# Saro00/DGN

Hardware: AMD Instinct MI355X
Metric: dgn_layer_fwd_bwd_edges_per_sec (higher is better)
Workload: dtype f32; 1 GPU; c2: ZINC-12k (12000 molecules, one batch), DGN towers: 5 towers, hidden 70, mean max min dir1-av dir1-dx x identity amplification attenuation; edges_per_gpu=586426, nodes_per_gpu=275167, parallelism=single GPU, step=edge weights + layer forward + backward

## Files before the change

dgn_amd/csrc/dgn_abi.hip:

```cpp
#include <hip/hip_runtime.h>

#include <atomic>
#include <cstdarg>
#include <cstdio>
#include <cstdlib>
#include <cstring>
#include <mutex>

#include "dgn_common.hpp"

namespace dgn {
namespace {
thread_local char g_err[512] = "";
}

void set_error(const char* fmt, ...) {
    va_list ap;
    va_start(ap, fmt);
    vsnprintf(g_err, sizeof(g_err), fmt, ap);
    va_end(ap);
}

namespace {
__global__ void zero_rows_kernel(int64_t rows, int64_t width, int64_t ld, float* __restrict__ p) {
// ... 30 lines not shown
hipError_t allow_lds(LdsOptIn& done, int bytes, const void* const* kernels, int n_kernels) {
    int dev = 0;
    hipError_t e = hipGetDevice(&dev);
    if (e != hipSuccess) return e;
    const unsigned long long bit = dev >= 0 && dev < 64 ? 1ull << dev : 0;
    if (done.load(std::memory_order_acquire) & bit) return hipSuccess;
    for (int i = 0; i < n_kernels; ++i) {
        e = hipFuncSetAttribute(kernels[i], hipFuncAttributeMaxDynamicSharedMemorySize, bytes);
        if (e != hipSuccess) return e;
    }
    done.fetch_or(bit, std::memory_order_release);
    return hipSuccess;
}

int n_cus() {
    static int cus = 0;
    if (!cus) {
        int dev = 0;
        hipDeviceProp_t prop;
        if (hipGetDevice(&dev) != hipSuccess || hipGetDeviceProperties(&prop, dev) != hipSuccess) return 256;
        cus = prop.multiProcessorCount > 0 ? prop.multiProcessorCount : 256;
    }
    return cus;
}

int hip_fail(hipError_t e, const char* what) {
    set_error("HIP error %d (%s) in %s", (int)e, hipGetErrorString(e), what);
    return DGN_ERR_HIP;
}
}

namespace dgn {
namespace {
struct OptDef { const char* name; const char* env; int64_t def; bool presence; };
const OptDef kOpts[OPT_COUNT] = {
    {"blk_lds_kb", "DGN_BLK_LDS_KB", 13, false},
    {"blk_min_nodes", "DGN_BLK_MIN_NODES", 131072, false},
    {"bwd_rows_per_wave", "DGN_BWD_ROWS_PER_WAVE", 4, false},
    {"tile_gemm", "DGN_TILE_GEMM", -1, false},
    {"tile_wgrad", "DGN_TILE_WGRAD", -1, false},
    {"no_zmask", "DGN_NO_ZMASK", 0, true},
    {"linear_small_min_waves", "DGN_LINEAR_SMALL_MIN_WAVES", 8, false},
    {"graph_bwd_tiles", "DGN_GRAPH_BWD_TILES", 0, false},
    {"odd_direct", "DGN_ODD_DIRECT", 1, false},
    {"bn_from_wgrad", "DGN_BN_FROM_WGRAD", 1, false},
    {"mix_bwd_fused", "DGN_MIX_BWD_FUSED", 1, false},
    {"blk_lds_pad_kb", "DGN_BLK_LDS_PAD_KB", 0, false},
    {"lin_wreg", "DGN_LIN_WREG", 3, false},
    {"bd_bwd_fused", "DGN_BD_BWD_FUSED", 1, false},
    {"bn_stats_fused", "DGN_BN_STATS_FUSED", 1, false},
    {"ew_big_min", "DGN_EW_BIG_MIN", 1 << 19, false},
    {"ew_separate", "DGN_EW_SEPARATE", 0, true},
    {"ew_no_flat8", "DGN_EW_NO_FLAT8", 0, true},
};
std::atomic<int64_t> g_opt[OPT_COUNT];
std::once_flag g_opt_once;
void init_options() {
    for (int i = 0; i < OPT_COUNT; ++i) {
        const char* e = getenv(kOpts[i].env);
        g_opt[i].store(e ? (kOpts[i].presence ? 1 : atoll(e)) : kOpts[i].def, std::memory_order_relaxed);
    }
    if (getenv("DGN_NO_MIX_FUSED")) g_opt[OPT_NO_ZMASK].store(1, std::memory_order_relaxed);
}
int find_option(const char* name) {
    if (name)
        for (int i = 0; i < OPT_COUNT; ++i)
            if (!strcmp(name, kOpts[i].name)) return i;
    return -1;
}
}
int64_t option(Opt o) {
    std::call_once(g_opt_once, init_options);
    return g_opt[o].load(std::memory_order_relaxed);
}
}

extern "C" int dgn_set_option(const char* name, int64_t value) {
    const int i = dgn::find_option(name);
    if (i < 0) { dgn::set_error("dgn_set_option: unknown option '%s'", name ? name : "(null)"); return DGN_ERR_INVALID; }
    std::call_once(dgn::g_opt_once, dgn::init_options);
    dgn::g_opt[i].store(value, std::memory_order_relaxed);
    return DGN_OK;
}
extern "C" int64_t dgn_get_option(const char* name) {
    const int i = dgn::find_option(name);
    if (i < 0) { dgn::set_error("dgn_get_option: unknown option '%s'", name ? name : "(null)"); return INT64_MIN; }
    return dgn::option(static_cast<dgn::Opt>(i));
}

extern "C" int dgn_abi_version(void) { return DGN_ABI_VERSION; }
extern "C" size_t dgn_sizeof(const char* name) {
#define DGN_SZ(T) if (name && !strcmp(name, #T)) return sizeof(T);
    DGN_SZ(DgnGraph) DGN_SZ(DgnChannel) DGN_SZ(DgnAggSpec) DGN_SZ(DgnMsg) DGN_SZ(DgnMsgGrad) DGN_SZ(DgnBnGrad) DGN_SZ(DgnTowersLayer)
    DGN_SZ(DgnTowersGrads) DGN_SZ(DgnDegreeClasses) DGN_SZ(DgnDcLayout) DGN_SZ(DgnDenseLayer) DGN_SZ(DgnDenseGrads) DGN_SZ(DgnBlockTable)
    DGN_SZ(DgnBlockLayer) DGN_SZ(DgnBlockGrads) DGN_SZ(DgnCollate)
#undef DGN_SZ
    return 0;
}
extern "C" const char* dgn_last_error(void) { return dgn::g_err; }
```

dgn_amd/csrc/dgn_common.hpp:

```cpp
#pragma once
#include <hip/hip_runtime.h>
#include <stdint.h>

#include <atomic>

#include "dgn_hip.h"

namespace dgn {

constexpr int kWave = 64;
#ifndef DGN_WAVES_PER_BLOCK
#define DGN_WAVES_PER_BLOCK 1
#endif
constexpr int kWavesPerBlock = DGN_WAVES_PER_BLOCK;
constexpr int kBlock = kWave * kWavesPerBlock;
constexpr int kXcds = 8;

void set_error(const char* fmt, ...);
enum Opt { OPT_BLK_LDS_KB, OPT_BLK_MIN_NODES, OPT_BWD_ROWS_PER_WAVE, OPT_TILE_GEMM, OPT_TILE_WGRAD, OPT_NO_ZMASK, OPT_LINEAR_SMALL_MIN_WAVES, OPT_GRAPH_BWD_TILES, OPT_ODD_DIRECT, OPT_BN_FROM_WGRAD, OPT_MIX_BWD_FUSED, OPT_BLK_LDS_PAD_KB, OPT_LIN_WREG, OPT_BD_BWD_FUSED, OPT_BN_STATS_FUSED, OPT_EW_BIG_MIN, OPT_EW_SEPARATE, OPT_EW_NO_FLAT8, OPT_COUNT };
int64_t option(Opt o);
int hip_fail(hipError_t e, const char* what);
int zero_rows_async(float* p, int64_t rows, int64_t width, int64_t ld, hipStream_t stream);
int scale_rows_async(int64_t n_rows, int32_t width, const float* g, int64_t ld_g, const float* g_loss, float* out, int64_t ld_out, hipStream_t stream);

using LdsOptIn = std::atomic<unsigned long long>;
hipError_t allow_lds(LdsOptIn& done, int bytes, const void* const* kernels, int n_kernels);
template <class... K>
inline hipError_t allow_lds(LdsOptIn& done, int bytes, K*... kernels) {
    const void* const list[] = {reinterpret_cast<const void*>(kernels)...};
    return allow_lds(done, bytes, list, (int)sizeof...(K));
}
int n_cus();
inline bool al16(const void* q) { return (reinterpret_cast<uintptr_t>(q) & 15) == 0; }

struct SlotSplit { int groups; int64_t per; int64_t bound; };
inline SlotSplit slot_split(int64_t n, int64_t min_per, int64_t max_groups) {
    int64_t g = (n + min_per - 1) / min_per;
    if (g > max_groups) g = max_groups;
    if (g < 1) g = 1;
    int64_t per = (n + g - 1) / g;
    if (per < 1) per = 1;
    return {(int)((n + per - 1) / per), per, g};
}
int scale_combine_backward_impl(int64_t n_nodes, int32_t T, int32_t S, int32_t fo, const float* g_y, int64_t ld_gy, const float* scale,
                                const float* row_scale, float* g_z, float* g_bias, void* ws, size_t ws_bytes, const DgnBnGrad* bn,
                                void* stream, int set_bias);

int scale_combine_forward_stats(int64_t n_nodes, int32_t T, int32_t S, int32_t fo, const float* z, const float* scale, const float* bias,
                                const float* row_scale, float* y, int64_t ld_y, double* part, size_t part_bytes, int* slots, void* stream);
int bn_tail_forward_nbt(int64_t n_rows, int32_t F, const float* x, int64_t ld, const float* gamma, const float* beta, float* running_mean,
                        float* running_var, float momentum, float eps, int32_t training, int32_t relu, const float* residual, float* y,
                        float* save_mean, float* save_invstd, void* ws, size_t ws_bytes, const int64_t* n_valid, int64_t* nbt, int32_t n_nbt,
                        void* stream);

int bn_tail_forward_from_partials(int64_t n_rows, int32_t F, int32_t G, const double* part, const float* x, int64_t ld, const float* gamma, const float* beta,
                                  float* running_mean, float* running_var, float momentum, float eps, int32_t relu, const float* residual, float* y,
                                  float* save_mean, float* save_invstd, int64_t* nbt, int32_t n_nbt, void* stream);
int bn_finalize_launch(int64_t n_rows, int32_t F, int32_t G, const double* part, float* running_mean, float* running_var, float momentum, float eps,
                       float* save_mean, float* save_invstd, int64_t* nbt, int32_t n_nbt, void* stream);

namespace dc {
size_t gemm_stats_bytes(int32_t n);
int gemm_stats(const DgnDegreeClasses* d, int32_t k, int32_t n, int32_t towers, const float* a, int64_t lda, int64_t a_tower, const float* w, int64_t ldw,
               int64_t class_stride, int64_t w_tower, const float* bias, const float* row_scale, float* c, int64_t ldc, int64_t c_tower, int32_t stream_out,
               double* part, size_t part_bytes, int* slots, void* stream);
}
namespace lin {
size_t combine_forward_stats_bytes(int32_t n_towers, int32_t f_out);
int combine_forward_stats(int64_t n_rows, int32_t k, int32_t n_towers, int32_t n_scalers, int32_t f_out, const float* a, int64_t stride_a,
                          const float* w, int64_t ldw, int64_t stride_w, const float* scale, const float* bias, const float* row_scale, float* y,
                          int64_t ld_y, double* part, size_t part_bytes, int* groups, void* stream);
int combine_backward_weight_bias_pick(int64_t n_rows, int32_t n_towers, int32_t n_scalers, int32_t f_out, int32_t k, const float* gy,
                                      int64_t stride_gy, const float* scale, const float* a, int64_t stride_a, float* dw, int64_t lddw,
                                      int64_t stride_dw, float* g_sum, float* pick, int32_t pick_slot, void* ws, size_t ws_bytes, void* stream);
int bd_backward_both_launch(int64_t n_rows, int32_t n_towers, int32_t f_in, const float* g, const float* w, int64_t ldw, const float* x,
                            const float* add1, const float* add2, float* g_h, float* dw, int64_t lddw, float* dbias, void* ws, size_t ws_bytes,
                            void* stream);
}

#define DGN_HIP_CHECK(expr)                                         \
    do {                                                            \
        hipError_t _e = (expr);                                     \
        if (_e != hipSuccess) return ::dgn::hip_fail(_e, #expr);    \
    } while (0)


__device__ __forceinline__ int lane_id() { return threadIdx.x & (kWave - 1); }

__device__ __forceinline__ int bcast_i(int v, int lane) { return __builtin_amdgcn_readlane(v, lane); }
__device__ __forceinline__ float bcast_f(float v, int lane) {
    return __int_as_float(__builtin_amdgcn_readlane(__float_as_int(v), lane));
}
__device__ __forceinline__ int uniform_i(int v) { return __builtin_amdgcn_readfirstlane(v); }

__device__ __forceinline__ int64_t xcd_remap(int64_t b, int64_t n_logical) {
#ifdef DGN_EXP_NOREMAP
    return b < n_logical ? b : -1;
#endif
    int64_t per = (n_logical + kXcds - 1) / kXcds;
    int64_t logical = (b % kXcds) * per + b / kXcds;
    return logical < n_logical ? logical : -1;
}
inline int64_t xcd_grid(int64_t n_logical) { return ((n_logical + kXcds - 1) / kXcds) * kXcds; }

template <int VEC>
__device__ __forceinline__ void ldv(float (&d)[VEC], const float* p) {
    if constexpr (VEC == 4) {
        float4 t = *reinterpret_cast<const float4*>(p);
        d[0] = t.x; d[1] = t.y; d[2] = t.z; d[3] = t.w;
    } else if constexpr (VEC == 2) {
        float2 t = *reinterpret_cast<const float2*>(p);
        d[0] = t.x; d[1] = t.y;
    } else {
        d[0] = *p;
    }
}
template <int VEC>
__device__ __forceinline__ void stv(float* p, const float (&d)[VEC]) {
    if constexpr (VEC == 4) {
        *reinterpret_cast<float4*>(p) = make_float4(d[0], d[1], d[2], d[3]);
    } else if constexpr (VEC == 2) {
        *reinterpret_cast<float2*>(p) = make_float2(d[0], d[1]);
    } else {
        *p = d[0];
    }
}
typedef float nt_f4 __attribute__((ext_vector_type(4)));
typedef float nt_f2 __attribute__((ext_vector_type(2)));
__device__ __forceinline__ void lds_add_f64(double* p, double v) {
    __hip_atomic_fetch_add((__attribute__((address_space(3))) double*)p, v, __ATOMIC_RELAXED, __HIP_MEMORY_SCOPE_WORKGROUP);
// ... 75 lines not shown
```

dgn_amd/csrc/dgn_edge_weights.hip:

```cpp
#include <hip/hip_runtime.h>

#include <cmath>
#include <cstdlib>

#include "dgn_common.hpp"

namespace dgn {
namespace {

struct EwParams {
    const int32_t* indptr;
    const int32_t* src;
    int64_t n_nodes;
    int64_t row_base;
    int32_t hub_threshold;
    int32_t hub_chunk;
    const int32_t* hub_rows;
    const int32_t* hub_chunk_ptr;
    const int32_t* chunk_hub;
    int64_t n_hub;
    int64_t n_chunks;
    const float* eig;
    const float* eig_s;
    const float* eig_d;
// ... 104 lines not shown
#pragma unroll
        for (int c = 0; c < DGN_MAX_CH; ++c) {
            if (c < p.n_ch) {
                const float d = dl[c];
                p.w[(int64_t)c * p.ld_w + e] = d;
                st[c].sabs += fabsf(d);
                st[c].spos += fmaxf(d, 0.f);
                st[c].sneg += fmaxf(-d, 0.f);
                st[c].mx = fmaxf(st[c].mx, p.ch[c].alpha * fabsf(d));
            }
        }
    }
#pragma unroll
    for (int c = 0; c < DGN_MAX_CH; ++c) {
        if (c < p.n_ch) {
            st[c].sabs = wave_sum(st[c].sabs);
            st[c].spos = wave_sum(st[c].spos);
            st[c].sneg = wave_sum(st[c].sneg);
            st[c].mx = wave_max(st[c].mx);
        }
    }
    if (any_softmax) {
        for (int e = beg + lane; e < end; e += kWave) {
#pragma unroll
            for (int c = 0; c < DGN_MAX_CH; ++c)
                if (c < p.n_ch && p.ch[c].kind == DGN_W_SOFTMAX)
                    st[c].se += expf(p.ch[c].alpha * fabsf(p.w[(int64_t)c * p.ld_w + e]) - st[c].mx);
        }
#pragma unroll
        for (int c = 0; c < DGN_MAX_CH; ++c)
            if (c < p.n_ch && p.ch[c].kind == DGN_W_SOFTMAX) st[c].se = wave_sum(st[c].se);
    }
}

__device__ __forceinline__ void range_write(const Stats (&st)[DGN_MAX_CH], const EwParams& p, int row, int beg, int end) {
    const int lane = lane_id();
    for (int e = beg + lane; e < end; e += kWave) {
#pragma unroll
        for (int c = 0; c < DGN_MAX_CH; ++c) {
            if (c < p.n_ch) {
                float* q = p.w + (int64_t)c * p.ld_w + e;
                *q = weight_of(p.ch[c], st[c], *q);
            }
        }
    }
}

constexpr int kFlatMax = 4;
constexpr int kGroup = 16;

template <int FM>
__device__ __forceinline__ void ew_flat_body(const EwParams& p, int64_t row64);
__global__ __launch_bounds__(256) void ew_rows_flat(const EwParams p) { ew_flat_body<kFlatMax>(p, (int64_t)blockIdx.x * blockDim.x + threadIdx.x); }
__global__ __launch_bounds__(256) void ew_rows_flat8(const EwParams p) { ew_flat_body<8>(p, (int64_t)blockIdx.x * blockDim.x + threadIdx.x); }
template <int FM>
__device__ __forceinline__ void ew_flat_body(const EwParams& p, int64_t row64) {
    if (row64 >= p.n_nodes) return;
    const int row = (int)row64;
    const int beg = p.indptr[row], end = p.indptr[row + 1];
    const int deg = end - beg;
    if (deg == 0 || deg > FM) return;
    RowEig re;
    re.load(p, row);
    float dl[FM][DGN_MAX_CH];
#pragma unroll
    for (int j = 0; j < FM; ++j) {
#pragma unroll
        for (int c = 0; c < DGN_MAX_CH; ++c) dl[j][c] = 0.f;
        if (j < deg) edge_deltas(dl[j], p, re, beg + j);
    }
#pragma unroll
    for (int c = 0; c < DGN_MAX_CH; ++c) {
        if (c >= p.n_ch) break;
        Stats st{0.f, 0.f, 0.f, -INFINITY, 0.f};
#pragma unroll
        for (int j = 0; j < FM; ++j) {
            if (j < deg) {
                const float d = dl[j][c];
                st.sabs += fabsf(d); st.spos += fmaxf(d, 0.f); st.sneg += fmaxf(-d, 0.f);
                st.mx = fmaxf(st.mx, p.ch[c].alpha * fabsf(d));
            }
        }
        if (p.ch[c].kind == DGN_W_SOFTMAX) {
#pragma unroll
            for (int j = 0; j < FM; ++j)
                if (j < deg) st.se += expf(p.ch[c].alpha * fabsf(dl[j][c]) - st.mx);
        }
#pragma unroll
        for (int j = 0; j < FM; ++j)
            if (j < deg) p.w[(int64_t)c * p.ld_w + beg + j] = weight_of(p.ch[c], st, dl[j][c]);
    }
}

__device__ __forceinline__ float group_sum(float v) {
#pragma unroll
    for (int o = kGroup / 2; o > 0; o >>= 1) v += __shfl_xor(v, o, kGroup);
    return v;
}
__device__ __forceinline__ float group_max(float v) {
#pragma unroll
    for (int o = kGroup / 2; o > 0; o >>= 1) v = fmaxf(v, __shfl_xor(v, o, kGroup));
    return v;
}

template <int R>
__device__ __forceinline__ int class_rows(const EwParams& p, int64_t base, int lo, int hi, int* list, int& my_beg, int& my_deg) {
// ... 142 lines not shown
    const int lane = lane_id();
    const int k0 = p.hub_chunk_ptr[hub], k1 = p.hub_chunk_ptr[hub + 1];
#pragma unroll
    for (int c = 0; c < DGN_MAX_CH; ++c) {
        float sabs = 0.f, spos = 0.f, sneg = 0.f, mx = -INFINITY;
        for (int k = k0 + lane; k < k1; k += kWave) {
            const float* s = p.slice_stats + ((int64_t)k * DGN_MAX_CH + c) * 5;
            sabs += s[0]; spos += s[1]; sneg += s[2];
            mx = fmaxf(mx, s[3]);
        }
        sabs = wave_sum(sabs); spos = wave_sum(spos); sneg = wave_sum(sneg); mx = wave_max(mx);
        float se = 0.f;
        for (int k = k0 + lane; k < k1; k += kWave) {
            const float* s = p.slice_stats + ((int64_t)k * DGN_MAX_CH + c) * 5;
            if (s[3] > -INFINITY) se += s[4] * expf(s[3] - mx);
        }
        se = wave_sum(se);
        if (lane == 0) {
            float* o = p.hub_stats + ((int64_t)hub * DGN_MAX_CH + c) * 5;
            o[0] = sabs; o[1] = spos; o[2] = sneg; o[3] = mx; o[4] = se;
        }
    }
}

__global__ __launch_bounds__(kBlock) void ew_hub_slice_write(const EwParams p) {
    const int64_t chunk64 = (int64_t)blockIdx.x * kWavesPerBlock + (threadIdx.x >> 6);
    if (chunk64 >= p.n_chunks) return;
    const int chunk = uniform_i((int)chunk64);
    int hub, row, beg, end;
    slice_bounds(p, chunk, hub, row, beg, end);
    Stats st[DGN_MAX_CH];
    const float* s = p.hub_stats + (int64_t)hub * DGN_MAX_CH * 5;
#pragma unroll
    for (int c = 0; c < DGN_MAX_CH; ++c) st[c] = Stats{s[c * 5 + 0], s[c * 5 + 1], s[c * 5 + 2], s[c * 5 + 3], s[c * 5 + 4]};
    range_write(st, p, row, beg, end);
}

size_t ws_bytes_for(const DgnGraph* g) {
    if (!g || g->n_hub <= 0) return 0;
    auto up = [](size_t x) { return (x + 255) & ~(size_t)255; };
    return up((size_t)g->n_chunks * DGN_MAX_CH * 5 * sizeof(float)) + up((size_t)g->n_hub * DGN_MAX_CH * 5 * sizeof(float));
}

}
}

using namespace dgn;

extern "C" size_t dgn_edge_weights_workspace_bytes(const DgnGraph* g, int32_t n_ch) {
    (void)n_ch;
    return ws_bytes_for(g);
}

extern "C" int dgn_edge_weights(const DgnGraph* g, const float* eig, const float* eig_s_edge, const float* eig_d_edge,
                                int64_t ld_eig, int32_t n_ch, const DgnChannel* ch, float* w, int64_t ld_w, void* ws,
                                size_t ws_bytes, void* stream_) {
    if (!g || !ch || !w) { set_error("null graph/channels/output"); return DGN_ERR_INVALID; }
    if (n_ch < 1 || n_ch > DGN_MAX_CH) { set_error("n_ch=%d outside 1..%d", n_ch, DGN_MAX_CH); return DGN_ERR_INVALID; }
    if (!eig && !(eig_s_edge && eig_d_edge)) { set_error("need eig, or eig_s_edge and eig_d_edge"); return DGN_ERR_INVALID; }
    if (g->n_nodes > INT32_MAX - 1 || g->n_edges > INT32_MAX - 1) { set_error("graph outside the int32 CSR range"); return DGN_ERR_INVALID; }
    if (ld_w < g->n_edges) { set_error("ld_w smaller than n_edges"); return DGN_ERR_INVALID; }
    for (int c = 0; c < n_ch; ++c) {
        if (ch[c].kind < DGN_W_ABSNORM || ch[c].kind > DGN_W_SOFTMAX) { set_error("unknown channel kind %d", ch[c].kind); return DGN_ERR_INVALID; }
        if (ch[c].eig_col < 0 || ch[c].eig_col >= ld_eig) { set_error("channel %d: eig column %d outside 0..%lld", c, ch[c].eig_col, (long long)ld_eig - 1); return DGN_ERR_INVALID; }
    }
    if (g->n_nodes == 0 || g->n_edges == 0) return DGN_OK;
    if (g->n_hub > 0 && (!ws || ws_bytes < ws_bytes_for(g))) { set_error("workspace too small: need %zu bytes", ws_bytes_for(g)); return DGN_ERR_WORKSPACE; }
    hipStream_t stream = static_cast<hipStream_t>(stream_);
    EwParams p{};
    p.indptr = g->indptr; p.src = g->src; p.n_nodes = g->n_nodes; p.row_base = g->row_base;
    p.n_hub = g->n_hub; p.n_chunks = g->n_hub > 0 ? g->n_chunks : 0;
    p.hub_threshold = g->n_hub > 0 ? g->hub_threshold : INT32_MAX;
    p.hub_chunk = g->hub_chunk; p.hub_rows = g->hub_rows; p.hub_chunk_ptr = g->hub_chunk_ptr; p.chunk_hub = g->chunk_hub;
    if (eig_s_edge && eig_d_edge) { p.eig_s = eig_s_edge; p.eig_d = eig_d_edge; } else { p.eig = eig; }
    p.ld_eig = ld_eig; p.n_ch = n_ch;
    int max_col = 0;
    for (int c = 0; c < n_ch; ++c) { p.ch[c] = ch[c]; max_col = ch[c].eig_col > max_col ? ch[c].eig_col : max_col; }
    p.n_need = max_col + 1 < 8 ? max_col + 1 : 8;
    {
        auto ok = [&](int v) {
            auto al = [&](const float* q) { return !q || (reinterpret_cast<uintptr_t>(q) % (4 * v)) == 0; };
            return ld_eig % v == 0 && al(eig) && al(eig_s_edge) && al(eig_d_edge);
        };
        p.vw = ok(4) ? 4 : (ok(2) ? 2 : 1);
    }
    p.w = w; p.ld_w = ld_w;
    if (g->n_hub > 0) {
        auto up = [](size_t x) { return (x + 255) & ~(size_t)255; };
        p.slice_stats = static_cast<float*>(ws);
        p.hub_stats = reinterpret_cast<float*>(static_cast<char*>(ws) + up((size_t)g->n_chunks * DGN_MAX_CH * 5 * sizeof(float)));
    }
    const int64_t big_min = option(OPT_EW_BIG_MIN);
    const bool big = p.n_nodes >= big_min;
    const bool no_merge = option(OPT_EW_SEPARATE) != 0;
    const bool no_flat8 = option(OPT_EW_NO_FLAT8) != 0;
    if (!no_flat8 && g->max_in_degree > kFlatMax && g->max_in_degree <= 8) {
        hipLaunchKernelGGL(ew_rows_flat8, dim3((unsigned)((p.n_nodes + 255) / 256)), dim3(256), 0, stream, p);
    } else if (!big && !no_merge && (g->max_in_degree == 0 || g->max_in_degree > kFlatMax)) {
        const int nf = (int)((p.n_nodes + kWave - 1) / kWave), ng = (int)((p.n_nodes + 3) / 4);
        const bool rows = g->max_in_degree == 0 || g->max_in_degree > kGroup;
        hipLaunchKernelGGL(ew_rows_small, dim3((unsigned)(nf + ng + (rows ? p.n_nodes : 0))), dim3(kWave), 0, stream, p, nf, ng);
    } else {
    hipLaunchKernelGGL(ew_rows_flat, dim3((unsigned)((p.n_nodes + 255) / 256)), dim3(256), 0, stream, p);
    if (g->max_in_degree == 0 || g->max_in_degree > kFlatMax)
    {
        if (big) hipLaunchKernelGGL(ew_rows_g16<kWave>, dim3((unsigned)((p.n_nodes + kWave - 1) / kWave)), dim3(kWave), 0, stream, p);
        else hipLaunchKernelGGL(ew_rows_g16<kWave / kGroup>, dim3((unsigned)((p.n_nodes + 3) / 4)), dim3(kWave), 0, stream, p);
    }
    if (g->max_in_degree == 0 || g->max_in_degree > kGroup) {
        if (big) hipLaunchKernelGGL(ew_rows<kWave>, dim3((unsigned)((p.n_nodes + kWave - 1) / kWave)), dim3(kWave), 0, stream, p);
        else hipLaunchKernelGGL(ew_rows<1>, dim3((unsigned)p.n_nodes), dim3(kWave), 0, stream, p);
    }
    }
    if (p.n_hub > 0) {
        const unsigned ns = (unsigned)((p.n_chunks + kWavesPerBlock - 1) / kWavesPerBlock);
        hipLaunchKernelGGL(ew_hub_slice_stats, dim3(ns), dim3(kBlock), 0, stream, p);
        hipLaunchKernelGGL(ew_hub_combine, dim3((unsigned)p.n_hub), dim3(kWave), 0, stream, p);
        hipLaunchKernelGGL(ew_hub_slice_write, dim3(ns), dim3(kBlock), 0, stream, p);
    }
    DGN_HIP_CHECK(hipGetLastError());
    return DGN_OK;
}
```

dgn_amd/csrc/dgn_linear.hip:

```cpp
#include "dgn_linear_kernels.hpp"

namespace dgn {
namespace lin {

hipError_t launch_linear_plain(int nt, int kb, const LinParams& p, int threads, size_t lds, hipStream_t st) {
    return launch_linear_grid<kPlain>(nt, kb, p, threads, lds, st);
}

namespace {
bool aligned8(const void* p) { return (reinterpret_cast<uintptr_t>(p) & 7) == 0; }

LinLauncher* const kLaunchers[kLinModes] = {launch_linear_plain, launch_linear_combine, launch_linear_expand, launch_linear_bn, launch_linear_act,
                                            launch_linear_add,   launch_linear_mix,     launch_linear_actm,   launch_linear_bnb};

LinParams lin_params(int64_t M, int k, int n, int T, const float* A, const float* W, int64_t ldw, int w_kn, float* C) {
    LinParams p{};
    p.M = M; p.k = k; p.n = n; p.T = T;
    p.A = A; p.W = W; p.ldw = ldw; p.w_kn = w_kn; p.C = C;
    return p;
}
LinParams combine_params(int64_t M, int k, int T, int S, int fo, const float* a, int64_t stride_a, const float* w, int64_t ldw, int64_t stride_w,
                         const float* scale, const float* bias, const float* row_scale, float* y, int64_t ld_y) {
    LinParams p = lin_params(M, k, S * fo, T, a, w, ldw, 0, nullptr);
    p.sA = stride_a; p.sW = stride_w;
// ... 169 lines not shown

extern "C" int dgn_linear_combine_forward(int64_t n_rows, int32_t k, int32_t n_towers, int32_t n_scalers, int32_t f_out,
                                          const float* a, int64_t stride_a, const float* w, int64_t ldw, int64_t stride_w,
                                          const float* scale, const float* bias, const float* row_scale, float* y, int64_t ld_y,
                                          void* stream) {
    const char* fn = "dgn_linear_combine_forward";
    const int n = n_scalers * f_out;
    if (n_rows < 0 || n_towers < 1 || n_scalers < 1 || n_scalers > 3 || f_out < 1 || !dgn_linear_supported(k, n, 0)) {
        set_error("%s: need even k and n_scalers * f_out in [2, 160], at most 3 scalers (k=%d n=%d)", fn, k, n);
        return -1;
    }
    if (n_rows == 0) return 0;
    if (!a || !w || !y || (n_scalers > 1 && !scale)) { set_error("%s: null operand", fn); return -1; }
    if ((f_out & 1) || (ld_y & 1) || !aligned8(y)) { set_error("%s: f_out and ld_y must be even, y 8-byte aligned", fn); return -1; }
    if ((stride_a & 1) || !aligned8(a) || ld_y < (int64_t)n_towers * f_out) { set_error("%s: A entries must be 8-byte aligned, y rows n_towers * f_out wide", fn); return -1; }
    LinParams p = combine_params(n_rows, k, n_towers, n_scalers, f_out, a, stride_a, w, ldw, stride_w, scale, bias, row_scale, y, ld_y);
    return launch_linear(fn, kCombine, p, stream);
}

size_t dgn::lin::combine_forward_stats_bytes(int32_t n_towers, int32_t f_out) {
    return (size_t)2 * n_towers * f_out * std::max(1, n_cus() * 32) * sizeof(double);
}

int dgn::lin::combine_forward_stats(int64_t n_rows, int32_t k, int32_t n_towers, int32_t n_scalers, int32_t f_out, const float* a, int64_t stride_a,
                                    const float* w, int64_t ldw, int64_t stride_w, const float* scale, const float* bias, const float* row_scale,
                                    float* y, int64_t ld_y, double* part, size_t part_bytes, int* groups, void* stream) {
    const char* fn = "combine_forward_stats";
    const int n = n_scalers * f_out;
    if (n_rows <= 0 || n_towers < 1 || n_scalers < 1 || n_scalers > 3 || f_out < 2 || (f_out & 1) || !dgn_linear_supported(k, n, 0) || kStrip * (f_out >> 1) > 256 ||
        !a || !w || !y || (n_scalers > 1 && !scale) || (ld_y & 1) || !aligned8(y) || (stride_a & 1) || !aligned8(a) || ld_y != (int64_t)n_towers * f_out || !part ||
        part_bytes < combine_forward_stats_bytes(n_towers, f_out))
        return 1;
    LinParams p = combine_params(n_rows, k, n_towers, n_scalers, f_out, a, stride_a, w, ldw, stride_w, scale, bias, row_scale, y, ld_y);
    p.bn_part = part; p.bn_F = n_towers * f_out;
    const int rc = launch_linear(fn, kCombine, p, stream);
    if (rc == 0) *groups = p.groups;
    return rc;
}

static int wgrad_groups(int64_t n_rows, int32_t k, int32_t n, int32_t batch) {
    const int64_t n_strips = (n_rows + kStrip - 1) / kStrip;
    const int per_cu = ((n + 15) / 16) * ((k + 15) / 16) <= 25 ? 2 : 1;
    int groups = std::max(1, n_cus() * per_cu / batch);
    return (int)std::max<int64_t>(1, std::min<int64_t>(groups, (n_strips + 3) / 4));
}

extern "C" size_t dgn_linear_wgrad_workspace_bytes(int64_t n_rows, int32_t k, int32_t n, int32_t batch) {
    if (n_rows <= 0 || batch < 1 || !dgn_linear_supported(k, n, 1)) return 0;
    const size_t NT = (n + 15) / 16, KT = (k + 15) / 16;
    return (size_t)batch * wgrad_groups(n_rows, k, n, batch) * NT * 16 * KT * 16 * sizeof(float);
}

static int launch_wgrad(const char* fn, WgParams& p, float* dw, int64_t lddw, int64_t stride_dw, float* dbias, int64_t stride_dbias,
                        void* ws, size_t ws_bytes, void* stream, float* pick = nullptr, int pick_off = 0, int pick_w = 0) {
    hipStream_t st = static_cast<hipStream_t>(stream);
    const int n = p.n, k = p.k, batch = p.T;
    const size_t need = dgn_linear_wgrad_workspace_bytes(p.M, k, n, batch);
    if (!ws || ws_bytes < need) { set_error("%s: workspace too small (%zu < %zu)", fn, ws_bytes, need); return -1; }
    p.part = static_cast<float*>(ws);
    p.groups = wgrad_groups(p.M, k, n, batch);
    p.ones = dbias != nullptr;
    const int NT = (n + 15) / 16, KT = (k + 15) / 16;
    if (p.bn_mean) p.bn_off = wgrad_bn_off(NT, KT, n, k, p.g_mask != nullptr);
    const size_t lds = wgrad_lds_bytes(NT, KT, n, k, p.g_mask != nullptr, p.bn_mean != nullptr);
    const hipError_t e = p.ex.gy ? launch_wgrad_expand(NT, KT, p, lds, st) : (p.g_mask ? launch_wgrad_gmask(NT, KT, p, lds, st) : launch_wgrad_plain(NT, KT, p, lds, st));
    DGN_HIP_CHECK(e);
    const int64_t total = (int64_t)batch * n * (dbias ? k + 1 : k);
    hipLaunchKernelGGL(ts_wgrad_finalize, dim3((unsigned)((total + 63) / 64)), dim3(64 * wg::kSumWaves), 0, st, batch, n, k, p.groups,
                       NT * 16, KT * 16, p.part, dw, lddw, stride_dw, dbias, stride_dbias, dbias ? pick : nullptr, pick_off, pick_w);
    DGN_HIP_CHECK(hipGetLastError());
    return 0;
}

static int zero_wgrad(float* dw, int64_t lddw, int64_t stride_dw, float* dbias, int64_t stride_dbias, int k, int n, int batch,
                      hipStream_t st) {
    for (int t = 0; t < batch; ++t) {
        if (zero_rows_async(dw + t * stride_dw, n, k, lddw, st)) return DGN_ERR_HIP;
        if (dbias && zero_rows_async(dbias + t * stride_dbias, 1, n, n, st)) return DGN_ERR_HIP;
    }
    return 0;
}

static int wgrad_open(const char* fn, int64_t n_rows, int k, int n, int batch, float* dw, int64_t lddw, int64_t stride_dw, float* dbias,
                      int64_t stride_dbias, void* stream) {
    if (dbias && k % 16 == 0) { set_error("%s: the bias gradient rides in X's padding column (k %% 16 != 0)", fn); return -1; }
    if (n_rows < 0 || batch < 1 || !dgn_linear_supported(k, n, 1)) { set_error("%s: need even k, n in [2, 160] and at most 45 tiles (k=%d n=%d)", fn, k, n); return -1; }
    if (!dw) { set_error("%s: null output", fn); return -1; }
    return n_rows == 0 ? zero_wgrad(dw, lddw, stride_dw, dbias, stride_dbias, k, n, batch, static_cast<hipStream_t>(stream)) : 1;
}
static WgParams wg_params(int64_t M, int k, int n, int T, const float* G, const float* X) {
    WgParams p{};
    p.M = M; p.n = n; p.k = k; p.T = T; p.G = G; p.X = X;
    return p;
}

extern "C" int dgn_linear_wgrad(int64_t n_rows, int32_t k, int32_t n, int32_t batch, const float* g, int64_t ldg,
                                int64_t stride_g, const float* x, int64_t ldx, int64_t stride_x, float* dw, int64_t lddw,
                                int64_t stride_dw, float* dbias, int64_t stride_dbias, void* ws, size_t ws_bytes,
                                void* stream) {
    const char* fn = "dgn_linear_wgrad";
    if (const int rc = wgrad_open(fn, n_rows, k, n, batch, dw, lddw, stride_dw, dbias, stride_dbias, stream); rc != 1) return rc;
    if (!g || !x) { set_error("%s: null operand", fn); return -1; }
    if (ldg != n || ldx != k || (stride_g & 1) || (stride_x & 1) || !aligned8(g) || !aligned8(x)) {
        set_error("%s: G and X must have dense rows (ldg == n, ldx == k) and 8-byte aligned batch entries", fn);
        return -1;
    }
    WgParams p = wg_params(n_rows, k, n, batch, g, x);
    p.sG = stride_g; p.sX = stride_x;
    return launch_wgrad(fn, p, dw, lddw, stride_dw, dbias, stride_dbias, ws, ws_bytes, stream);
}

extern "C" int dgn_linear_wgrad_bn(int64_t n_rows, int32_t k, int32_t n, const float* g, const float* x, float* dw, int64_t lddw, float* dbias,
                                   const float* bn_mean, const float* bn_invstd, const float* bn_gamma, const float* bn_beta, void* ws,
                                   size_t ws_bytes, void* stream) {
    const char* fn = "dgn_linear_wgrad_bn";
    if (const int rc = wgrad_open(fn, n_rows, k, n, 1, dw, lddw, 0, dbias, 0, stream); rc != 1) return rc;
    if (!g || !x || !bn_mean || !bn_invstd || !aligned8(g) || !aligned8(x)) { set_error("%s: null or misaligned operand", fn); return -1; }
    WgParams p = wg_params(n_rows, k, n, 1, g, x);
    p.bn_mean = bn_mean; p.bn_invstd = bn_invstd; p.bn_gamma = bn_gamma; p.bn_beta = bn_beta;
    return launch_wgrad(fn, p, dw, lddw, 0, dbias, 0, ws, ws_bytes, stream);
}

// ... 10 lines not shown
    p.g_mask = zmask; p.act_kind = act; p.act_slope = slope;
    p.bn_mean = bn_mean; p.bn_invstd = bn_invstd; p.bn_gamma = bn_gamma; p.bn_beta = bn_beta;
    return launch_wgrad(fn, p, dw, lddw, 0, dbias, 0, ws, ws_bytes, stream);
}

static bool expand_ok(const char* fn, int64_t n_rows, int32_t n_towers, int32_t n_scalers, int32_t f_out, const float* gy,
                      int64_t stride_gy, const float* scale) {
    if (n_rows < 0 || n_towers < 1 || n_scalers < 1 || n_scalers > 3 || f_out < 2 || (f_out & 1)) {
        set_error("%s: need 1..3 scalers and an even f_out", fn);
        return false;
    }
    if (n_rows > 0 && (!gy || (n_scalers > 1 && !scale) || (stride_gy & 1) || !aligned8(gy))) {
        set_error("%s: gy must be [n_towers][n_rows][f_out] with 8-byte aligned towers; scale is required for more than one scaler", fn);
        return false;
    }
    return true;
}

extern "C" int dgn_linear_combine_backward_input(int64_t n_rows, int32_t n_towers, int32_t n_scalers, int32_t f_out, int32_t k,
                                                 const float* gy, int64_t stride_gy, const float* scale, const float* w, int64_t ldw,
                                                 int64_t stride_w, float* g_a, int64_t stride_ga, void* stream) {
    const char* fn = "dgn_linear_combine_backward_input";
    const int red = n_scalers * f_out;
    if (!expand_ok(fn, n_rows, n_towers, n_scalers, f_out, gy, stride_gy, scale)) return -1;
    if (!dgn_linear_supported(red, k, 0)) { set_error("%s: need even widths in [2, 160] (S*f_out=%d k=%d)", fn, red, k); return -1; }
    if (n_rows == 0) return 0;
    if (!w || !g_a || (stride_ga & 1) || !aligned8(g_a)) { set_error("%s: null or misaligned operand", fn); return -1; }
    LinParams p = lin_params(n_rows, red, k, n_towers, nullptr, w, ldw, 1, g_a);
    p.sW = stride_w; p.sC = stride_ga;
    if (n_scalers == 1) { p.A = gy; p.sA = stride_gy; }
    else p.ex = ExpandSrc{gy, stride_gy, scale, n_scalers, f_out};
    return launch_linear(fn, n_scalers == 1 ? kPlain : kExpand, p, stream);
}

extern "C" int dgn_linear_combine_backward_weight(int64_t n_rows, int32_t n_towers, int32_t n_scalers, int32_t f_out, int32_t k,
                                                  const float* gy, int64_t stride_gy, const float* scale, const float* a,
                                                  int64_t stride_a, float* dw, int64_t lddw, int64_t stride_dw, void* ws,
                                                  size_t ws_bytes, void* stream) {
    return dgn_linear_combine_backward_weight_bias(n_rows, n_towers, n_scalers, f_out, k, gy, stride_gy, scale, a, stride_a, dw, lddw, stride_dw,
                                                   nullptr, ws, ws_bytes, stream);
}

extern "C" int dgn_linear_combine_backward_weight_bias(int64_t n_rows, int32_t n_towers, int32_t n_scalers, int32_t f_out, int32_t k,
                                                       const float* gy, int64_t stride_gy, const float* scale, const float* a,
                                                       int64_t stride_a, float* dw, int64_t lddw, int64_t stride_dw, float* g_sum,
                                                       void* ws, size_t ws_bytes, void* stream) {
    return dgn::lin::combine_backward_weight_bias_pick(n_rows, n_towers, n_scalers, f_out, k, gy, stride_gy, scale, a, stride_a, dw, lddw, stride_dw, g_sum,
                                                       nullptr, 0, ws, ws_bytes, stream);
}

int dgn::lin::combine_backward_weight_bias_pick(int64_t n_rows, int32_t n_towers, int32_t n_scalers, int32_t f_out, int32_t k, const float* gy,
                                                int64_t stride_gy, const float* scale, const float* a, int64_t stride_a, float* dw, int64_t lddw,
                                                int64_t stride_dw, float* g_sum, float* pick, int32_t pick_slot, void* ws, size_t ws_bytes,
                                                void* stream) {
    const char* fn = "dgn_linear_combine_backward_weight";
    if (g_sum && k % 16 == 0) { set_error("%s: the column sums ride in A's padding column (k %% 16 != 0)", fn); return -1; }
    const int n = n_scalers * f_out;
    if (!expand_ok(fn, n_rows, n_towers, n_scalers, f_out, gy, stride_gy, scale)) return -1;
    if (!dgn_linear_supported(k, n, 1)) { set_error("%s: need even widths in [2, 160] and at most 45 tiles (k=%d S*f_out=%d)", fn, k, n); return -1; }
    if (!dw) { set_error("%s: null output", fn); return -1; }
    if (n_rows == 0) {
        if (pick && zero_rows_async(pick, 1, (int64_t)n_towers * f_out, (int64_t)n_towers * f_out, static_cast<hipStream_t>(stream))) return DGN_ERR_HIP;
        return zero_wgrad(dw, lddw, stride_dw, g_sum, n, k, n, n_towers, static_cast<hipStream_t>(stream));
    }
    if (!a || (stride_a & 1) || !aligned8(a)) { set_error("%s: null or misaligned operand", fn); return -1; }
    WgParams p = wg_params(n_rows, k, n, n_towers, nullptr, a);
    p.sX = stride_a;
    if (n_scalers == 1) { p.G = gy; p.sG = stride_gy; }
    else p.ex = ExpandSrc{gy, stride_gy, scale, n_scalers, f_out};
    if (pick && (!g_sum || pick_slot < 0 || pick_slot >= n_scalers)) { set_error("%s: pick needs g_sum and a scaler slot", fn); return -1; }
    return launch_wgrad(fn, p, dw, lddw, stride_dw, g_sum, n, ws, ws_bytes, stream, pick, pick_slot * f_out, f_out);
}
```

dgn_amd/csrc/dgn_linear_bd.hip:

```cpp
#include "dgn_linear_kernels.hpp"

namespace dgn {
namespace lin {

struct BdParams {
    int64_t M;
    int T, fi;
    const float* A;
    const float* X;
    const float* W; int64_t ldw;
    const float* bias;
    float* C;
    const float* add1; const float* add2;
    float* part;
    int groups;
};

constexpr int bd_fwd_threads(int T, int FB) { return T * FB <= 3 ? 1024 : (T * FB <= 6 ? 768 : (T * FB <= 8 ? 512 : 256)); }
constexpr int bd_bwd_threads(int T, int FB) { return T * FB <= 2 ? 1024 : (T * FB <= 5 ? 512 : 256); }
constexpr int bd_wg_waves_per_simd(int T, int FB) { return 2 * T * FB * FB <= 10 ? 2 : 1; }

enum { kBdFwd = 0, kBdBwd = 1, kBdWg = 2, kBdBoth = 3 };
struct BdLayout { int bias, strips, wave, fold; };
constexpr BdLayout bd_layout(int which, int T, int fi) {
// ... 342 lines not shown
            if (u + 1 < T * 2 * FB) {
                const int t1 = (u + 1) / (2 * FB), j1 = ((u + 1) / FB) % 2, b1 = (u + 1) % FB;
                xn = bd_operand(xrow + j1 * n + t1 * fi + 16 * b1, fi - 16 * b1 - 4 * g);
#pragma unroll
                for (int q = 0; q < FB; ++q) wn[q] = *reinterpret_cast<const f4*>(Wl + ((t1 * FB + q) * 16 + m) * KP2 + j1 * 16 * FB + 16 * b1 + 4 * g);
            }
            __builtin_amdgcn_sched_barrier(0);
#pragma unroll
            for (int s = 0; s < 4; ++s)
#pragma unroll
                for (int q = 0; q < FB; ++q)
                    acc[t * FB + q] = __builtin_amdgcn_mfma_f32_16x16x4f32(wv[q][s], xv[s], acc[t * FB + q], 0, 0, 0);
            __builtin_amdgcn_sched_barrier(0);
        }
#pragma unroll
        for (int s = 0; s < 4; ++s) {
            const float* grow = U + (4 * g + s) * k2 + m;
            const float* xr = Xl + (4 * g + s) * n + m;
#pragma unroll
            for (int t = 0; t < T; ++t) {
                float xv[FB], gv[2 * FB];
#pragma unroll
                for (int b = 0; b < FB; ++b) {
                    xv[b] = xr[t * fi + 16 * b];
                    if (16 * b + m == fi) xv[b] = 1.f;
                }
#pragma unroll
                for (int ja = 0; ja < 2 * FB; ++ja) gv[ja] = grow[(ja / FB) * n + t * fi + 16 * (ja % FB)];
#pragma unroll
                for (int ja = 0; ja < 2 * FB; ++ja)
#pragma unroll
                    for (int b = 0; b < FB; ++b)
                        accw[(t * 2 * FB + ja) * FB + b] = __builtin_amdgcn_mfma_f32_16x16x4f32(gv[ja], xv[b], accw[(t * 2 * FB + ja) * FB + b], 0, 0, 0);
            }
            __builtin_amdgcn_sched_barrier(0);
        }
        float* c = U + m * n + 4 * g;
#pragma unroll
        for (int t = 0; t < T; ++t)
#pragma unroll
            for (int q = 0; q < FB; ++q) {
                const f4 v = acc[t * FB + q];
                const int col = 16 * q + 4 * g;
                float* d = c + t * fi + 16 * q;
                if (col < fi) *reinterpret_cast<float2*>(d) = make_float2(v[0], v[1]);
                if (col + 2 < fi) *reinterpret_cast<float2*>(d + 2) = make_float2(v[2], v[3]);
            }
        out_strip = strip;
    }
    if (out_strip >= 0) store_out();
    wg::wave_fold<NTW * 256>(lds, p.part, blockIdx.x, accw, [&](int q, int r) { return q * 256 + (4 * g + r) * 16 + m; });
}

static __global__ __launch_bounds__(64 * wg::kSumWaves) void bd_wgrad_finalize(int T, int fi, int FB, int slots, const float* __restrict__ part,
                                                                               float* __restrict__ dW, int64_t lddw, float* __restrict__ dbias) {
    __shared__ float red[wg::kSumWaves][64];
    const int Fm = T * fi, kk = Fm + 1, ntl = 2 * T * FB * FB;
    const int64_t e = (int64_t)blockIdx.x * 64 + (threadIdx.x & 63);
    const bool live = e < (int64_t)2 * Fm * kk;
    int r = 0, c = 0, off = 0;
    bool diag = false;
    if (live) {
        r = (int)(e / kk);
        c = (int)(e - (int64_t)r * kk);
        const int j = r / Fm, rr = r - j * Fm, t = rr / fi, a = rr - t * fi;
        const int b = c == Fm ? fi : c - t * fi;
        diag = c == Fm || (c >= t * fi && c < (t + 1) * fi);
        if (diag) off = (((t * 2 + j) * FB + (a >> 4)) * FB + (b >> 4)) * 256 + (a & 15) * 16 + (b & 15);
    }
    const float v = wg::slot_sum16(part + off, (int64_t)ntl * 256, slots, diag, red);
    if (live && threadIdx.x < 64) {
        if (c < Fm) dW[(int64_t)r * lddw + c] = v;
        else if (dbias) dbias[r] = v;
    }
}

namespace {
#define DGN_BD_SHAPES(X) X(5, 14) X(5, 10) X(5, 12) X(5, 18) X(5, 20) X(5, 22) X(5, 24) X(5, 26) X(5, 28) X(5, 30) X(4, 14) X(2, 14)

int bd_blocks(int T, int fi) {
#define DGN_CASE(TT, FF) if (T == TT && fi == FF) return (FF + 15) / 16;
    DGN_BD_SHAPES(DGN_CASE)
#undef DGN_CASE
    return 0;
}

template <int T, int FI>
hipError_t bd_launch_one(int which, const BdParams& p, int threads, size_t lds, hipStream_t st) {
    static_assert(FI % 2 == 0 && FI % 16 != 0 && T * FI <= 16 * kMaxTiles, "even widths with room for the ones column");
    static LdsOptIn lds_ok{0};
    hipError_t e;
    if constexpr (FI <= 16) e = allow_lds(lds_ok, kLdsBudget, &bd_forward<T, FI>, &bd_backward_input<T, FI>, &bd_wgrad<T, FI>, &bd_backward_both<T, FI>);
    else e = allow_lds(lds_ok, kLdsBudget, &bd_forward<T, FI>, &bd_backward_input<T, FI>, &bd_wgrad<T, FI>);
    if (e != hipSuccess) return e;
    if (which == kBdFwd) hipLaunchKernelGGL((bd_forward<T, FI>), dim3(p.groups), dim3(threads), lds, st, p);
    else if (which == kBdBwd) hipLaunchKernelGGL((bd_backward_input<T, FI>), dim3(p.groups), dim3(threads), lds, st, p);
    else if (which == kBdBoth) {
        if constexpr (FI <= 16) hipLaunchKernelGGL((bd_backward_both<T, FI>), dim3(p.groups), dim3(threads), lds, st, p);
        else return hipErrorInvalidValue;
    }
    else hipLaunchKernelGGL((bd_wgrad<T, FI>), dim3(p.groups), dim3(256), lds, st, p);
    return hipGetLastError();
}

hipError_t bd_launch(int which, const BdParams& p, int threads, size_t lds, hipStream_t st) {
#define DGN_CASE(TT, FF) if (p.T == TT && p.fi == FF) return bd_launch_one<TT, FF>(which, p, threads, lds, st);
    DGN_BD_SHAPES(DGN_CASE)
#undef DGN_CASE
    return hipErrorInvalidValue;
}

int bd_wgrad_groups(int64_t n_rows) {
    const int64_t n_strips = (n_rows + kStrip - 1) / kStrip;
    return (int)std::max<int64_t>(1, std::min<int64_t>(2 * n_cus(), (n_strips + 3) / 4));
}

int bd_launch_stream(const char* fn, int which, BdParams& p, void* stream) {
    const BdLayout L = bd_layout(which, p.T, p.fi);
    const int FB = bd_blocks(p.T, p.fi), max_waves = (which == kBdFwd ? bd_fwd_threads(p.T, FB) : bd_bwd_threads(p.T, FB)) / 64;
    int waves = 0, per_cu = 0;
    for (int w = max_waves; w >= 1; --w) {
        const size_t bytes = bd_lds_bytes(L, w);
        if (bytes > (size_t)kLdsBudget) continue;
        const int pc = std::min((int)(kLdsBudget / bytes), 16 / w);
        if (pc * w > per_cu * waves) { waves = w; per_cu = pc; }
    }
    if (!waves) { set_error("%s: operands do not fit in LDS", fn); return -1; }
    const int64_t n_strips = (p.M + kStrip - 1) / kStrip;
    p.groups = (int)std::max<int64_t>(1, std::min<int64_t>((int64_t)n_cus() * per_cu, (n_strips + waves - 1) / waves));
    DGN_HIP_CHECK(bd_launch(which, p, waves * 64, bd_lds_bytes(L, waves), static_cast<hipStream_t>(stream)));
    return 0;
}

int bd_finalize(const BdParams& p, float* dw, int64_t lddw, float* dbias, hipStream_t st) {
    const int Fm = p.T * p.fi;
    const int64_t total = (int64_t)2 * Fm * (Fm + 1);
    hipLaunchKernelGGL(bd_wgrad_finalize, dim3((unsigned)((total + 63) / 64)), dim3(64 * wg::kSumWaves), 0, st, p.T, p.fi, bd_blocks(p.T, p.fi), p.groups, p.part, dw,
                       lddw, dbias);
    DGN_HIP_CHECK(hipGetLastError());
    return DGN_OK;
}
}
}
}

using namespace dgn;
using namespace dgn::lin;

extern "C" int dgn_linear_bd_supported(int32_t n_towers, int32_t f_in) { return bd_blocks(n_towers, f_in) != 0; }

extern "C" int dgn_linear_bd_forward(int64_t n_rows, int32_t n_towers, int32_t f_in, const float* a, const float* w, int64_t ldw,
                                     const float* bias, float* c, void* stream) {
    const char* fn = "dgn_linear_bd_forward";
    if (n_rows < 0 || !bd_blocks(n_towers, f_in)) { set_error("%s: unsupported towers x width (%d x %d)", fn, n_towers, f_in); return DGN_ERR_INVALID; }
    if (n_rows == 0) return DGN_OK;
    if (!a || !w || !c || !al16(a) || !al16(c) || ldw < (int64_t)n_towers * f_in) { set_error("%s: null / misaligned operand (16-byte aligned dense rows)", fn); return DGN_ERR_INVALID; }
    BdParams p{};
    p.M = n_rows; p.T = n_towers; p.fi = f_in; p.A = a; p.W = w; p.ldw = ldw; p.bias = bias; p.C = c;
    return bd_launch_stream(fn, kBdFwd, p, stream);
}

extern "C" int dgn_linear_bd_backward_input(int64_t n_rows, int32_t n_towers, int32_t f_in, const float* g, const float* w, int64_t ldw,
                                            const float* add1, const float* add2, float* c, void* stream) {
    const char* fn = "dgn_linear_bd_backward_input";
    if (n_rows < 0 || !bd_blocks(n_towers, f_in)) { set_error("%s: unsupported towers x width (%d x %d)", fn, n_towers, f_in); return DGN_ERR_INVALID; }
    if (n_rows == 0) return DGN_OK;
    if (!g || !w || !c || !al16(g) || !al16(c) || (add1 && !al16(add1)) || (add2 && !al16(add2)) || (add2 && !add1) || ldw < (int64_t)n_towers * f_in) {
        set_error("%s: null / misaligned operand (16-byte aligned dense rows; add2 needs add1)", fn);
        return DGN_ERR_INVALID;
    }
    BdParams p{};
    p.M = n_rows; p.T = n_towers; p.fi = f_in; p.A = g; p.W = w; p.ldw = ldw; p.C = c; p.add1 = add1; p.add2 = add2;
    return bd_launch_stream(fn, kBdBwd, p, stream);
}

extern "C" size_t dgn_linear_bd_wgrad_workspace_bytes(int64_t n_rows, int32_t n_towers, int32_t f_in) {
    const int FB = bd_blocks(n_towers, f_in);
    if (n_rows <= 0 || !FB) return 0;
    return (size_t)bd_wgrad_groups(n_rows) * 2 * n_towers * FB * FB * 256 * sizeof(float);
}

extern "C" int dgn_linear_bd_wgrad(int64_t n_rows, int32_t n_towers, int32_t f_in, const float* g, const float* x, float* dw, int64_t lddw,
                                   float* dbias, void* ws, size_t ws_bytes, void* stream) {
    const char* fn = "dgn_linear_bd_wgrad";
    const int FB = bd_blocks(n_towers, f_in);
    if (n_rows < 0 || !FB) { set_error("%s: unsupported towers x width (%d x %d)", fn, n_towers, f_in); return DGN_ERR_INVALID; }
    const int Fm = n_towers * f_in;
    if (!dw || lddw < Fm) { set_error("%s: null output", fn); return DGN_ERR_INVALID; }
    hipStream_t st = static_cast<hipStream_t>(stream);
    if (n_rows == 0) {
        if (zero_rows_async(dw, 2 * Fm, Fm, lddw, st)) return DGN_ERR_HIP;
        if (dbias && zero_rows_async(dbias, 1, 2 * Fm, 2 * Fm, st)) return DGN_ERR_HIP;
        return DGN_OK;
    }
    if (!g || !x || !al16(g) || !al16(x)) { set_error("%s: null / misaligned operand (16-byte aligned dense rows)", fn); return DGN_ERR_INVALID; }
    const size_t need = dgn_linear_bd_wgrad_workspace_bytes(n_rows, n_towers, f_in);
    if (!ws || ws_bytes < need) { set_error("%s: workspace too small (%zu < %zu)", fn, ws_bytes, need); return DGN_ERR_WORKSPACE; }
    BdParams p{};
    p.M = n_rows; p.T = n_towers; p.fi = f_in; p.A = g; p.X = x; p.part = static_cast<float*>(ws);
    p.groups = bd_wgrad_groups(n_rows);
    DGN_HIP_CHECK(bd_launch(kBdWg, p, 256, bd_lds_bytes(bd_layout(kBdWg, n_towers, f_in), 256 / 64), st));
    return bd_finalize(p, dw, lddw, dbias, st);
}

namespace dgn {
namespace lin {
int bd_backward_both_launch(int64_t n_rows, int32_t n_towers, int32_t f_in, const float* g, const float* w, int64_t ldw, const float* x,
                            const float* add1, const float* add2, float* g_h, float* dw, int64_t lddw, float* dbias, void* ws, size_t ws_bytes,
                            void* stream) {
    const char* fn = "bd_backward_both";
    const int FB = bd_blocks(n_towers, f_in);
    const int Fm = n_towers * f_in;
    if (n_rows <= 0 || FB != 1 || !g || !w || !x || !g_h || !dw || !al16(g) || !al16(x) || !al16(g_h) || (add1 && !al16(add1)) || (add2 && !al16(add2)) ||
        (add2 && !add1) || ldw < Fm || lddw < Fm) {
        set_error("%s: unsupported shape or operand", fn);
        return DGN_ERR_INVALID;
    }
    const size_t need = dgn_linear_bd_wgrad_workspace_bytes(n_rows, n_towers, f_in);
    if (!ws || ws_bytes < need) { set_error("%s: workspace too small (%zu < %zu)", fn, ws_bytes, need); return DGN_ERR_WORKSPACE; }
    BdParams p{};
    p.M = n_rows; p.T = n_towers; p.fi = f_in; p.A = g; p.X = x; p.W = w; p.ldw = ldw; p.C = g_h; p.add1 = add1; p.add2 = add2;
    p.part = static_cast<float*>(ws);
    const BdLayout L = bd_layout(kBdBoth, n_towers, f_in);
    int waves = 8;
    while (waves > 1 && bd_lds_bytes(L, waves) > (size_t)kLdsBudget) waves /= 2;
    const size_t lds = bd_lds_bytes(L, waves);
    if (lds > (size_t)kLdsBudget) { set_error("%s: operands do not fit in LDS", fn); return DGN_ERR_INVALID; }
    const int64_t n_strips = (n_rows + kStrip - 1) / kStrip;
    p.groups = (int)std::max<int64_t>(1, std::min<int64_t>(std::min<int64_t>(n_cus(), bd_wgrad_groups(n_rows)), (n_strips + waves - 1) / waves));
    hipStream_t st = static_cast<hipStream_t>(stream);
    DGN_HIP_CHECK(bd_launch(kBdBoth, p, waves * 64, lds, st));
    return bd_finalize(p, dw, lddw, dbias, st);
}
}
}
```

dgn_amd/csrc/dgn_linear_kernels.hpp:

```cpp
#pragma once
#include <hip/hip_runtime.h>

#include <algorithm>

#include "dgn_common.hpp"
#include "dgn_wgrad.hpp"

namespace dgn {
namespace lin {

using f4 = __attribute__((ext_vector_type(4))) float;

constexpr int kStrip = 16;
constexpr int kMaxTiles = 10;
constexpr int kLdsBudget = 160 * 1024;
constexpr int kFacFloats = 2 * kStrip * 4;
constexpr int kMaxWgradTiles = 45;

__host__ __device__ inline int lds_stride(int k) { return ((k + 15) / 16) * 16 + 4; }

struct ExpandSrc {
    const float* gy; int64_t sT;
    const float* sc;
    int S, fo;
// ... 612 lines not shown
#pragma unroll
    for (int q = 0; q < NT * KT; ++q) acc[q] = f4{0.f, 0.f, 0.f, 0.f};

    const int i16 = lane & 15, mq = lane >> 4;
    if (first < n_strips) {
        fetch_g(first);
        load_strip<NLX>(px, X, p.M, k, first, lane);
    }
    for (int64_t strip = first; strip < n_strips; strip += step) {
        const int rows = (int)min((int64_t)kStrip, p.M - strip * kStrip);
        if constexpr (EXPAND) {
            store_expand<NLG>(Gl, Fl, pg, fac, p.ex, rows, lane);
        } else {
            if (rows < kStrip) {
#pragma unroll
                for (int j = 0; j < NLG; ++j)
                    if (strip_idx2(j, lane) >= rows * (n >> 1)) pg[j] = make_float2(0.f, 0.f);
            }
            if constexpr (GMASK) {
                asm volatile("s_waitcnt vmcnt(0)" ::: "memory");
                const unsigned short* mw = reinterpret_cast<const unsigned short*>(Ml + (buf ^ 1) * 2 * n);
                unsigned gmz[NLG / 2];
#pragma unroll
                for (int jq = 0; jq < NLG / 2; ++jq) gmz[jq] = mw[min(jq * 64 + lane, 4 * n - 1)];
                store_strip_mask<NLG>(Gl, pg, gmz, n, lane, p.act_kind, p.act_slope, nullptr, 0);
            } else {
                store_strip<NLG>(Gl, pg, n, lane);
            }
        }
        if (BnW) store_strip_bn<NLX>(Xl, px, k, lane, BnW, KT * 16);
        else store_strip<NLX>(Xl, px, k, lane);
        if (strip + step < n_strips) {
            fetch_g(strip + step);
            load_strip<NLX>(px, X, p.M, k, strip + step, lane);
        }
#pragma unroll
        for (int s = 0; s < 4; ++s) {
            float gv[NT], xv[KT];
#pragma unroll
            for (int a = 0; a < NT; ++a) gv[a] = Gl[(4 * mq + s) * n + 16 * a + i16];
#pragma unroll
            for (int b = 0; b < KT; ++b) xv[b] = Xl[(4 * mq + s) * k + 16 * b + i16];
            if (p.ones && 16 * (KT - 1) + i16 == k) xv[KT - 1] = 1.f;
#pragma unroll
            for (int a = 0; a < NT; ++a)
#pragma unroll
                for (int b = 0; b < KT; ++b) acc[a * KT + b] = __builtin_amdgcn_mfma_f32_16x16x4f32(gv[a], xv[b], acc[a * KT + b], 0, 0, 0);
        }
    }
    wg::wave_fold<NT * 16 * KT * 16>(lds, p.part, (int64_t)t * p.groups + grp, acc,
                                     [&](int q, int r) { return (16 * (q / KT) + 4 * mq + r) * (KT * 16) + 16 * (q % KT) + i16; });
}

static __global__ __launch_bounds__(64 * wg::kSumWaves) void ts_wgrad_finalize(int T, int n, int k, int slots, int npad, int kpad,
                                                         const float* __restrict__ part, float* __restrict__ dW,
                                                         int64_t lddw, int64_t sdW, float* __restrict__ dbias, int64_t sdb,
                                                         float* __restrict__ pick = nullptr, int pick_off = 0, int pick_w = 0) {
    __shared__ float red[wg::kSumWaves][64];
    const int kk = dbias ? k + 1 : k;
    const int64_t e = (int64_t)blockIdx.x * 64 + (threadIdx.x & 63);
    const bool live = e < (int64_t)T * n * kk;
    int t = 0, r = 0, c = 0;
    if (live) {
        t = (int)(e / ((int64_t)n * kk));
        const int rem = (int)(e - (int64_t)t * n * kk);
        r = rem / kk;
        c = rem - r * kk;
    }
    const float v = wg::slot_sum16(part + (int64_t)t * slots * npad * kpad + (int64_t)r * kpad + c, (int64_t)npad * kpad, slots, live, red);
    if (live && threadIdx.x < 64) {
        if (c < k) dW[(int64_t)t * sdW + (int64_t)r * lddw + c] = v;
        else {
            dbias[(int64_t)t * sdb + r] = v;
            if (pick && r >= pick_off && r < pick_off + pick_w) pick[t * pick_w + r - pick_off] = v;
        }
    }
}

constexpr bool linear_shape_ok(int NT, int KB, int mode) {
    return (!(mode == kActPlain || mode == kActMask || mode == kActMaskBnb) || 4 * NT + 8 * KB <= 104) &&
           (!(mode == kAddPlain || mode == kMixFwd || mode == kActMaskBnb) || 16 * NT + 4 * KB <= 128) &&
           (mode != kActMaskBnb || (NT <= 5 && KB <= 7 && NT + KB <= 11));
}
template <int NT, int KB, int MODE>
hipError_t launch_linear_nkm(const LinParams& p, int threads, size_t lds, hipStream_t st) {
    if constexpr (!linear_shape_ok(NT, KB, MODE)) {
        return hipErrorInvalidValue;
    } else {
    if constexpr (linear_wreg_ok(NT, KB, MODE)) {
        if (p.wreg) {
            static LdsOptIn lds_ok_w{0};
            if (hipError_t e = allow_lds(lds_ok_w, kLdsBudget, &ts_linear<NT, KB, MODE, true>)) return e;
            hipLaunchKernelGGL((ts_linear<NT, KB, MODE, true>), dim3(p.T * p.groups), dim3(threads), lds, st, p);
            return hipGetLastError();
        }
    }
    static LdsOptIn lds_ok{0};
    if (hipError_t e = allow_lds(lds_ok, kLdsBudget, &ts_linear<NT, KB, MODE>)) return e;
    hipLaunchKernelGGL((ts_linear<NT, KB, MODE>), dim3(p.T * p.groups), dim3(threads), lds, st, p);
    return hipGetLastError();
    }
}
template <int NT, int KT, bool EXPAND, bool GMASK = false>
hipError_t launch_wgrad_nke(const WgParams& p, size_t lds, hipStream_t st) {
    if constexpr (NT * KT > kMaxWgradTiles) {
        return hipErrorInvalidValue;
    } else {
        static LdsOptIn lds_ok{0};
        if (hipError_t e = allow_lds(lds_ok, kLdsBudget, &ts_wgrad<NT, KT, EXPAND, GMASK>)) return e;
        hipLaunchKernelGGL((ts_wgrad<NT, KT, EXPAND, GMASK>), dim3(p.T * p.groups), dim3(256), lds, st, p);
        return hipGetLastError();
    }
}

#define DGN_LIN_CASES(X) X(1) X(2) X(3) X(4) X(5) X(6) X(7) X(8) X(9) X(10)

template <int NT, int MODE>
hipError_t launch_linear_n(int kb, const LinParams& p, int threads, size_t lds, hipStream_t st) {
    switch (kb) {
#define DGN_CASE(K) case K: return launch_linear_nkm<NT, K, MODE>(p, threads, lds, st);
        DGN_LIN_CASES(DGN_CASE)
#undef DGN_CASE
    }
    return hipErrorInvalidValue;
}
template <int MODE>
hipError_t launch_linear_grid(int nt, int kb, const LinParams& p, int threads, size_t lds, hipStream_t st) {
    switch (nt) {
#define DGN_CASE(N) case N: return launch_linear_n<N, MODE>(kb, p, threads, lds, st);
// ... 34 lines not shown
```

dgn_amd/csrc/dgn_towers.hip:

```cpp
#include <hip/hip_runtime.h>
#include <algorithm>
#include <cstdlib>

#include <cstdint>

#include "dgn_common.hpp"

namespace dgn {
namespace {

inline size_t up256(size_t x) { return (x + 255) & ~(size_t)255; }

__global__ __launch_bounds__(256) void add3_rows(int64_t n4, const float4* __restrict__ res, const float4* __restrict__ a,
                                                 const float4* __restrict__ b, float4* __restrict__ out) {
    const int64_t i = (int64_t)blockIdx.x * blockDim.x + threadIdx.x;
    if (i >= n4) return;
    float4 v = a[i];
    const float4 w = b[i];
    v.x += w.x; v.y += w.y; v.z += w.z; v.w += w.w;
    if (res) {
        const float4 r = res[i];
        v.x += r.x; v.y += r.y; v.z += r.z; v.w += r.w;
    }
    out[i] = v;
}
__global__ __launch_bounds__(256) void add3_tail(int64_t first, int64_t n, const float* __restrict__ res, const float* __restrict__ a,
                                                 const float* __restrict__ b, float* __restrict__ out) {
    const int64_t i = first + (int64_t)blockIdx.x * blockDim.x + threadIdx.x;
    if (i >= n) return;
    out[i] = a[i] + b[i] + (res ? res[i] : 0.f);
}

__global__ __launch_bounds__(256) void assemble_params(int64_t n, const int64_t* __restrict__ ptrs, const int32_t* __restrict__ map_param,
                                                       const int32_t* __restrict__ map_off, float* __restrict__ out) {
    const int64_t i = (int64_t)blockIdx.x * blockDim.x + threadIdx.x;
    if (i >= n) return;
    const int q = map_param[i];
    out[i] = q < 0 ? 0.f : reinterpret_cast<const float*>(ptrs[q])[map_off[i]];
}

__global__ __launch_bounds__(64) void mix_bn_finalize(int Fo, const float* __restrict__ dwx, const float* __restrict__ db, const float* __restrict__ w,
                                                      int64_t ldw, const float* __restrict__ gamma, const float* __restrict__ beta,
                                                      float* __restrict__ g_w, int64_t ldgw, float* __restrict__ g_gamma, float* __restrict__ g_beta,
                                                      float* __restrict__ sums) {
    const int c = blockIdx.x, lane = threadIdx.x;
    const float ga = gamma ? gamma[c] : 1.f, be = beta ? beta[c] : 0.f;
    double s0 = 0.0, s1 = 0.0;
    for (int o = lane; o < Fo; o += 64) {
        const float x = dwx[(int64_t)o * Fo + c], b = db[o], wv = w[(int64_t)o * ldw + c];
        s0 += (double)b * (double)wv;
        s1 += (double)x * (double)wv;
        g_w[(int64_t)o * ldgw + c] = ga * x + be * b;
    }
#pragma unroll
    for (int d = 32; d >= 1; d >>= 1) {
        s0 += __shfl_xor(s0, d, 64);
        s1 += __shfl_xor(s1, d, 64);
    }
    if (lane == 0) {
        sums[c] = (float)s0; sums[Fo + c] = (float)s1;
        g_beta[c] = (float)s0; g_gamma[c] = (float)s1;
    }
}

struct Dims {
    int64_t N;
    int T, fi, fo, S, Fm, Fo, K;
};

bool dims_of(const DgnTowersLayer* L, Dims& d, const char* fn) {
    if (!L || !L->graph || !L->spec) { set_error("%s: null layer / graph / spec", fn); return false; }
    d.N = L->graph->n_nodes; d.T = L->n_towers; d.fi = L->f_in; d.fo = L->f_out; d.S = L->n_scalers;
    if (d.T < 1 || d.fi < 1 || d.fo < 1 || d.S < 1 || d.S > 3) { set_error("%s: bad tower / scaler counts", fn); return false; }
    d.Fm = d.T * d.fi; d.Fo = d.T * d.fo;
    const int a_total = L->spec->agg_total > 0 ? L->spec->agg_total : L->spec->n_agg;
    d.K = a_total * d.fi;
    if (L->spec->n_towers != d.T || L->spec->n_scalers != 1) { set_error("%s: the sweep spec must carry the towers and ONE (identity) scaler", fn); return false; }
    if (!dgn_linear_supported(d.Fm, 2 * d.Fm, 1) || !dgn_linear_supported(2 * d.Fm, d.Fm, 0) || !dgn_linear_supported(d.K, d.S * d.fo, 1) ||
        !dgn_linear_supported(d.S * d.fo, d.K, 0) || !dgn_linear_supported(d.Fo, d.Fo, 1) || (d.Fm % 16) == 0 || (d.fo & 1) || d.Fo > 1024) {
        set_error("%s: widths outside the streaming Linear kernels (in %d, towers %d x (%d -> %d), %d scalers)", fn, d.Fm, d.T, d.fi, d.fo, d.S);
        return false;
    }
    return true;
}

bool use_bd(const DgnTowersLayer* L, const Dims& d) {
    static const bool off = getenv("DGN_NO_BD") != nullptr;
    return !off && dgn_linear_bd_supported(d.T, d.fi) && ((reinterpret_cast<uintptr_t>(L->h) | reinterpret_cast<uintptr_t>(L->pq)) & 15) == 0;
}

DgnMsg sweep_msg(const DgnTowersLayer* L, const Dims& d) {
// ... 92 lines not shown
                                nullptr, L->y1, L->save_mean, L->save_invstd, ws, bn_ws, L->n_valid, L->num_batches_tracked, L->n_nbt, stream));
    }
    if (L->drop_p > 0.0f) DGN_TRY(dgn_dropout_forward(d.N * d.Fo, L->y1, L->drop_p, L->drop_seed, L->drop_offset, L->y1, L->drop_mask, stream));
    static const bool no_mix_fused = getenv("DGN_NO_MIX_FUSED") != nullptr;
    const bool al = ((reinterpret_cast<uintptr_t>(L->z) | reinterpret_cast<uintptr_t>(L->zmask) | reinterpret_cast<uintptr_t>(L->out) |
                      reinterpret_cast<uintptr_t>(L->h)) & 15) == 0;
    if (!L->y1 && !no_mix_fused && al && dgn_linear_add_supported(d.Fo, d.Fo)) {
        if (L->zmask) DGN_TRY(dgn_linear_forward_bn_act_mask(d.N, d.Fo, d.Fo, L->y0, L->w_mix, d.Fo, L->save_mean, L->save_invstd, L->bn_gamma, L->bn_beta,
                                                             L->b_mix, 2, L->slope, L->residual ? L->h : nullptr, L->zmask, L->out, stream));
        else DGN_TRY(dgn_linear_forward_bn_act(d.N, d.Fo, d.Fo, L->y0, L->w_mix, d.Fo, L->save_mean, L->save_invstd, L->bn_gamma, L->bn_beta, L->b_mix, 2,
                                               L->slope, L->residual ? L->h : nullptr, L->z, L->out, stream));
        return DGN_OK;
    }
    if (!L->z) { set_error("%s: zmask without the fused mixing-network kernel (operands 16-byte aligned, no y1): give z", fn); return DGN_ERR_INVALID; }
    if (L->y1) DGN_TRY(dgn_linear_forward(d.N, d.Fo, d.Fo, 1, L->y1, d.Fo, 0, L->w_mix, d.Fo, 0, 0, nullptr, 0, L->z, d.Fo, 0, stream));
    else DGN_TRY(dgn_linear_forward_bn(d.N, d.Fo, d.Fo, L->y0, L->w_mix, d.Fo, 0, nullptr, L->z, L->save_mean, L->save_invstd, L->bn_gamma,
                                       L->bn_beta, stream));
    DGN_TRY(dgn_bias_act_forward(d.N, d.Fo, L->z, d.Fo, L->b_mix, 2, L->slope, L->residual ? L->h : nullptr, L->out, stream));
    return DGN_OK;
}

namespace {
struct BwdScratch {
    size_t g_z, g_y1, sums, g_yr, g_aggx, g_pq, g_in, g_hpq, bn_ws, comb_ws, wg_mix, wg_post, wg_sd, agg_ws, dwx, g_sum, total;
};
BwdScratch bwd_scratch(const DgnTowersLayer* L, const Dims& d) {
    BwdScratch s{};
    size_t off = 0;
    auto take = [&](size_t bytes) { const size_t at = off; off += up256(bytes); return at; };
    const size_t NF = (size_t)d.N * d.Fo * 4;
    s.g_z = take(NF); s.g_y1 = take(NF); s.sums = take((size_t)2 * d.Fo * 4);
    s.g_yr = take(NF);
    s.g_aggx = take((size_t)d.T * d.N * d.K * 4);
    s.g_pq = take((size_t)d.N * 2 * d.Fm * 4); s.g_in = take((size_t)d.N * d.Fm * 4); s.g_hpq = take((size_t)d.N * d.Fm * 4);
    s.bn_ws = take(dgn_bn_tail_workspace_bytes(d.N, d.Fo));
    s.comb_ws = take(dgn_scale_combine_backward_workspace_bytes(d.N, d.T, d.fo));
    s.wg_mix = take(dgn_linear_wgrad_workspace_bytes(d.N, d.Fo, d.Fo, 1));
    s.wg_post = take(dgn_linear_wgrad_workspace_bytes(d.N, d.K, d.S * d.fo, d.T));
    s.wg_sd = take(std::max(dgn_linear_wgrad_workspace_bytes(d.N, d.Fm, 2 * d.Fm, 1), dgn_linear_bd_wgrad_workspace_bytes(d.N, d.T, d.fi)));
    s.agg_ws = take(dgn_agg_backward_workspace_bytes(L->graph, L->spec, d.Fm, 1));
    s.dwx = take((size_t)d.Fo * d.Fo * 4);
    s.g_sum = take((size_t)d.T * d.S * d.fo * 4);
    s.total = off;
    return s;
}
}

extern "C" size_t dgn_towers_layer_backward_workspace_bytes(const DgnTowersLayer* L) {
    Dims d;
    if (!dims_of(L, d, "dgn_towers_layer_backward_workspace_bytes")) return 0;
    return bwd_scratch(L, d).total;
}

extern "C" int dgn_towers_layer_backward(const DgnTowersLayer* L, const DgnTowersGrads* G, void* stream) {
    const char* fn = "dgn_towers_layer_backward";
    Dims d;
    if (!dims_of(L, d, fn)) return DGN_ERR_INVALID;
    if (!G) { set_error("%s: null grads", fn); return DGN_ERR_INVALID; }
    if (d.N == 0) return DGN_OK;
    if (!G->g_out || !G->g_h || !G->g_w_sd || !G->g_bias_sd || !G->g_w_post || !G->g_b_post || !G->g_gamma || !G->g_beta || !G->g_w_mix ||
        !G->g_b_mix) { set_error("%s: null gradient buffer", fn); return DGN_ERR_INVALID; }
    if (!drop_ok(L, fn, false)) return DGN_ERR_INVALID;
    const BwdScratch s = bwd_scratch(L, d);
    if (!L->ws || L->ws_bytes < s.total) { set_error("%s: workspace too small (%zu < %zu)", fn, L->ws_bytes, s.total); return DGN_ERR_WORKSPACE; }
    hipStream_t st = static_cast<hipStream_t>(stream);
    char* ws = static_cast<char*>(L->ws);
    auto f = [&](size_t off) { return reinterpret_cast<float*>(ws + off); };
    float *g_z = f(s.g_z), *g_y1 = f(s.g_y1), *sums = f(s.sums), *g_yr = f(s.g_yr), *g_aggx = f(s.g_aggx), *g_pq = f(s.g_pq),
          *g_in = f(s.g_in), *g_hpq = f(s.g_hpq);
    const bool fused_act = L->y1 == nullptr && d.Fo % 16 != 0 && (reinterpret_cast<uintptr_t>(g_z) & 15) == 0 && dgn_linear_act_supported(d.Fo, d.Fo);
    const bool bn_derived = fused_act && L->drop_p == 0.0f && !L->n_valid && option(OPT_BN_FROM_WGRAD) != 0;
    const bool mix_fused = bn_derived && L->zmask && (reinterpret_cast<uintptr_t>(L->zmask) & 15) == 0 && L->id_slot1 >= 1 && L->id_slot1 <= d.S && d.K % 16 != 0 && d.T <= 15 &&
                           (reinterpret_cast<uintptr_t>(L->y0) & 15) == 0 && dgn_linear_bnb_supported(d.Fo, d.Fo) && option(OPT_MIX_BWD_FUSED) != 0;
    if (mix_fused) {
        DGN_TRY(dgn_linear_wgrad_bn_act_mask(d.N, d.Fo, d.Fo, G->g_out, L->zmask, 2, L->slope, L->y0, f(s.dwx), d.Fo, G->g_b_mix, L->save_mean,
                                             L->save_invstd, nullptr, nullptr, ws + s.wg_mix, dgn_linear_wgrad_workspace_bytes(d.N, d.Fo, d.Fo, 1), stream));
        hipLaunchKernelGGL(mix_bn_finalize, dim3(d.Fo), dim3(64), 0, st, d.Fo, (const float*)f(s.dwx), (const float*)G->g_b_mix, L->w_mix, (int64_t)d.Fo,
                           L->bn_gamma, L->bn_beta, G->g_w_mix, (int64_t)d.Fo, G->g_gamma, G->g_beta, sums);
        DGN_HIP_CHECK(hipGetLastError());
        DGN_TRY(dgn_linear_forward_act_mask_bnb(d.N, d.Fo, d.Fo, G->g_out, L->zmask, 2, L->slope, L->w_mix, d.Fo, 1, L->y0, L->save_mean, L->save_invstd,
                                                L->bn_gamma, sums, L->snorm, d.fo, g_yr, d.N * d.fo, stream));
    } else if (fused_act) {
        if (L->zmask) DGN_TRY(dgn_linear_forward_act_mask(d.N, d.Fo, d.Fo, G->g_out, L->zmask, 2, L->slope, L->w_mix, d.Fo, 1, g_y1, g_z, stream));
        else DGN_TRY(dgn_linear_forward_act(d.N, d.Fo, d.Fo, G->g_out, L->z, L->b_mix, 2, L->slope, L->w_mix, d.Fo, 1, g_y1, g_z, stream));
        if (bn_derived) {
            DGN_TRY(dgn_linear_wgrad_bn(d.N, d.Fo, d.Fo, g_z, L->y0, f(s.dwx), d.Fo, G->g_b_mix, L->save_mean, L->save_invstd, nullptr, nullptr,
                                        ws + s.wg_mix, dgn_linear_wgrad_workspace_bytes(d.N, d.Fo, d.Fo, 1), stream));
            hipLaunchKernelGGL(mix_bn_finalize, dim3(d.Fo), dim3(64), 0, st, d.Fo, (const float*)f(s.dwx), (const float*)G->g_b_mix, L->w_mix, (int64_t)d.Fo,
                               L->bn_gamma, L->bn_beta, G->g_w_mix, (int64_t)d.Fo, G->g_gamma, G->g_beta, sums);
            DGN_HIP_CHECK(hipGetLastError());
        } else {
            DGN_TRY(dgn_linear_wgrad_bn(d.N, d.Fo, d.Fo, g_z, L->y0, G->g_w_mix, d.Fo, G->g_b_mix, L->save_mean, L->save_invstd, L->bn_gamma, L->bn_beta,
                                        ws + s.wg_mix, dgn_linear_wgrad_workspace_bytes(d.N, d.Fo, d.Fo, 1), stream));
        }
    } else {
        if (!L->z) { set_error("%s: zmask without the fused activation-gradient kernel: give z", fn); return DGN_ERR_INVALID; }
        DGN_TRY(dgn_bias_act_backward(d.N, d.Fo, G->g_out, L->z, d.Fo, L->b_mix, 2, L->slope, g_z, G->g_b_mix, ws + s.bn_ws,
                                      dgn_bn_tail_workspace_bytes(d.N, d.Fo), stream));
        DGN_TRY(dgn_linear_forward(d.N, d.Fo, d.Fo, 1, g_z, d.Fo, 0, L->w_mix, d.Fo, 0, 1, nullptr, 0, g_y1, d.Fo, 0, stream));
        if (L->y1) DGN_TRY(dgn_linear_wgrad(d.N, d.Fo, d.Fo, 1, g_z, d.Fo, 0, L->y1, d.Fo, 0, G->g_w_mix, d.Fo, 0, nullptr, 0, ws + s.wg_mix,
                                            dgn_linear_wgrad_workspace_bytes(d.N, d.Fo, d.Fo, 1), stream));
        else DGN_TRY(dgn_linear_wgrad_bn(d.N, d.Fo, d.Fo, g_z, L->y0, G->g_w_mix, d.Fo, nullptr, L->save_mean, L->save_invstd, L->bn_gamma, L->bn_beta,
                                         ws + s.wg_mix, dgn_linear_wgrad_workspace_bytes(d.N, d.Fo, d.Fo, 1), stream));
    }
    if (L->drop_p > 0.0f) DGN_TRY(dgn_dropout_backward(d.N * d.Fo, g_y1, L->drop_mask, L->drop_p, g_y1, stream));
    if (!bn_derived)
        DGN_TRY(dgn_bn_tail_backward(d.N, d.Fo, g_y1, L->y0, d.Fo, L->bn_gamma, L->bn_beta, L->save_mean, L->save_invstd, 0, nullptr, G->g_gamma,
                                     G->g_beta, sums, ws + s.bn_ws, dgn_bn_tail_workspace_bytes(d.N, d.Fo), L->n_valid, stream));
    if (!mix_fused) {
        DgnBnGrad bn{};
        bn.g_out = g_y1; bn.y = L->y0; bn.ld = d.Fo; bn.gamma = L->bn_gamma; bn.beta = L->bn_beta; bn.mean = L->save_mean; bn.invstd = L->save_invstd;
        bn.sums = sums; bn.relu = 0; bn.n_valid = L->n_valid;
        DGN_TRY(scale_combine_backward_impl(d.N, d.T, 1, d.fo, nullptr, 0, nullptr, L->snorm, g_yr, G->g_b_post, ws + s.comb_ws,
                                           dgn_scale_combine_backward_workspace_bytes(d.N, d.T, d.fo), &bn, stream, 1));
    }
    DGN_TRY(dgn_linear_combine_backward_input(d.N, d.T, d.S, d.fo, d.K, g_yr, d.N * d.fo, L->scale, L->w_post, d.K, (int64_t)d.S * d.fo * d.K,
                                              g_aggx, d.N * d.K, stream));
    float* g_sum = mix_fused ? f(s.g_sum) : nullptr;
    DGN_TRY(lin::combine_backward_weight_bias_pick(d.N, d.T, d.S, d.fo, d.K, g_yr, d.N * d.fo, L->scale, L->aggx, d.N * d.K, G->g_w_post, d.K,
                                                   (int64_t)d.S * d.fo * d.K, g_sum, mix_fused ? G->g_b_post : nullptr, mix_fused ? L->id_slot1 - 1 : 0,
                                                   ws + s.wg_post, dgn_linear_wgrad_workspace_bytes(d.N, d.K, d.S * d.fo, d.T), stream));
    const DgnMsg msg = sweep_msg(L, d);
    DgnMsgGrad gr{};
    gr.g_src = g_pq; gr.ld_src = 2 * d.Fm;
    gr.g_dst = g_pq + d.Fm; gr.ld_dst = 2 * d.Fm;
    gr.g_in = g_in; gr.ld_in = d.Fm;
    gr.accumulate = 0;
    DGN_TRY(dgn_agg_backward_aux(L->graph, L->spec, &msg, L->w, L->ld_w, L->log_deg, g_aggx, d.K, L->agg_aux, &gr, ws + s.agg_ws,
                                 dgn_agg_backward_workspace_bytes(L->graph, L->spec, d.Fm, 1), stream));
    const float* res = L->residual ? G->g_out : nullptr;
    static const bool no_add_epilogue = getenv("DGN_NO_ADD_EPILOGUE") != nullptr;
    const bool al = ((reinterpret_cast<uintptr_t>(G->g_h) | reinterpret_cast<uintptr_t>(G->g_out)) & 15) == 0;
    const bool fused_add = !no_add_epilogue && al && (reinterpret_cast<uintptr_t>(g_in) & 15) == 0 && dgn_linear_add_supported(2 * d.Fm, d.Fm);
    if (use_bd(L, d) && al && ((reinterpret_cast<uintptr_t>(g_in) | reinterpret_cast<uintptr_t>(g_pq)) & 15) == 0) {
        if (option(OPT_BD_BWD_FUSED) && d.fi <= 16 && (reinterpret_cast<uintptr_t>(L->h) & 15) == 0) {
            DGN_TRY(lin::bd_backward_both_launch(d.N, d.T, d.fi, g_pq, L->w_sd, d.Fm, L->h, g_in, res, G->g_h, G->g_w_sd, d.Fm, G->g_bias_sd, ws + s.wg_sd,
                                                 dgn_linear_bd_wgrad_workspace_bytes(d.N, d.T, d.fi), stream));
            return DGN_OK;
        }
        DGN_TRY(dgn_linear_bd_backward_input(d.N, d.T, d.fi, g_pq, L->w_sd, d.Fm, g_in, res, G->g_h, stream));
        DGN_TRY(dgn_linear_bd_wgrad(d.N, d.T, d.fi, g_pq, L->h, G->g_w_sd, d.Fm, G->g_bias_sd, ws + s.wg_sd,
                                    dgn_linear_bd_wgrad_workspace_bytes(d.N, d.T, d.fi), stream));
        return DGN_OK;
    }
    if (fused_add) DGN_TRY(dgn_linear_forward_add(d.N, 2 * d.Fm, d.Fm, g_pq, L->w_sd, d.Fm, 1, g_in, res, G->g_h, stream));
    else DGN_TRY(dgn_linear_forward(d.N, 2 * d.Fm, d.Fm, 1, g_pq, 2 * d.Fm, 0, L->w_sd, d.Fm, 0, 1, nullptr, 0, g_hpq, d.Fm, 0, stream));
    DGN_TRY(dgn_linear_wgrad(d.N, d.Fm, 2 * d.Fm, 1, g_pq, 2 * d.Fm, 0, L->h, d.Fm, 0, G->g_w_sd, d.Fm, 0, G->g_bias_sd, 0, ws + s.wg_sd,
                             dgn_linear_wgrad_workspace_bytes(d.N, d.Fm, 2 * d.Fm, 1), stream));
    if (fused_add) return DGN_OK;
    const int64_t n = d.N * d.Fm, n4 = n / 4;
    if (al && n4 > 0) {
        hipLaunchKernelGGL(add3_rows, dim3((unsigned)((n4 + 255) / 256)), dim3(256), 0, st, n4, reinterpret_cast<const float4*>(res),
                           reinterpret_cast<const float4*>(g_in), reinterpret_cast<const float4*>(g_hpq), reinterpret_cast<float4*>(G->g_h));
        if (n > 4 * n4) hipLaunchKernelGGL(add3_tail, dim3(1), dim3(256), 0, st, 4 * n4, n, res, g_in, g_hpq, G->g_h);
    } else {
        hipLaunchKernelGGL(add3_tail, dim3((unsigned)((n + 255) / 256)), dim3(256), 0, st, (int64_t)0, n, res, g_in, g_hpq, G->g_h);
    }
    DGN_HIP_CHECK(hipGetLastError());
    return DGN_OK;
}

extern "C" int dgn_assemble_params(int64_t n_out, const int64_t* param_ptrs, const int32_t* map_param, const int32_t* map_off, float* out,
                                   void* stream) {
    if (n_out < 0 || (n_out > 0 && (!param_ptrs || !map_param || !map_off || !out))) { set_error("dgn_assemble_params: null argument"); return DGN_ERR_INVALID; }
    if (n_out == 0) return DGN_OK;
    hipLaunchKernelGGL(assemble_params, dim3((unsigned)((n_out + 255) / 256)), dim3(256), 0, static_cast<hipStream_t>(stream), n_out, param_ptrs,
                       map_param, map_off, out);
    DGN_HIP_CHECK(hipGetLastError());
    return DGN_OK;
}
```

dgn_amd/dgn_layer.py:

```python
from __future__ import annotations

import math

from typing import List, Sequence

import torch
import torch.nn as nn
import torch.nn.functional as F

from .graph import DGNGraph, as_dgn_graph
from .layers import MLP, FCLayer
from . import ops as _ops
from .ops import (bn_tail, bn_tail_fused, bn_tail_supported, combine_bn_tail, directional_aggregate, linear_combine_bn_tail,
                  linear_combine_supported, node_linear, scale_combine, towers_layer, towers_layer_supported)
from .spec import (AGGREGATOR_NAMES, SCALE_AMPLIFICATION, SCALE_IDENTITY, SCALER_NAMES, X_IN_NAME, make_plan,
                   parse_aggregator, parse_scaler)


class _Named:

    def __init__(self, name: str):
        self.name = name

    def __repr__(self):
# ... 519 lines not shown
        return out

    def _linked_bn_stats(self, dev):
        bns = [t.batchnorm_h for t in self.towers]
        fo = self.output_tower
        link = self.__dict__.get("_bn_link")
        if link is not None and link[0].device == dev and all(
                b.running_mean.data_ptr() == link[0].data_ptr() + 4 * i * fo and b.running_var.data_ptr() == link[1].data_ptr() + 4 * i * fo
                and b.num_batches_tracked.data_ptr() == link[2].data_ptr() + 8 * i for i, b in enumerate(bns)):
            return link
        with torch.no_grad():
            rm = torch.cat([b.running_mean.reshape(-1) for b in bns]).to(dev)
            rv = torch.cat([b.running_var.reshape(-1) for b in bns]).to(dev)
            nbt = torch.stack([b.num_batches_tracked.reshape(()) for b in bns]).to(dev)
            for i, b in enumerate(bns):
                b.running_mean, b.running_var = rm[i * fo:(i + 1) * fo], rv[i * fo:(i + 1) * fo]
                b.num_batches_tracked = nbt[i]
        self.__dict__["_bn_link"] = (rm, rv, nbt)
        return self.__dict__["_bn_link"]

    def _assemble(self, plist):
        T, fi, fo = len(self.towers), self.input_tower, self.output_tower
        w_pre, b_pre = torch.stack(plist[0::6]), torch.stack(plist[1::6])
        w_post, b_post = torch.stack(plist[2::6]), torch.stack(plist[3::6])
        dev, dt = w_pre.device, w_pre.dtype
        Fm = T * fi
        ops = {}
        if self.divide_input:
            idx = torch.arange(T, device=dev)
            bd = torch.zeros(2, T, fi, T, fi, dtype=dt, device=dev)
            bd[:, idx, :, idx, :] = torch.stack([w_pre[:, :, :fi], w_pre[:, :, fi:2 * fi]], dim=1)
            ops["w_sd"] = bd.view(2 * Fm, Fm)
        else:
            ops["w_sd"] = torch.cat([w_pre[:, :, :fi].reshape(Fm, fi), w_pre[:, :, fi:2 * fi].reshape(Fm, fi)], dim=0)
        ops["bias_sd"] = torch.cat([torch.zeros(Fm, dtype=dt, device=dev), b_pre.reshape(Fm)])
        if self.edge_features:
            ops["w_edge"] = w_pre[:, :, 2 * fi:].reshape(Fm, -1)
        ops["b_p"] = b_post.reshape(T * fo)
        ops["bn_gamma"], ops["bn_beta"] = torch.cat(plist[4::6]), torch.cat(plist[5::6])
        S = self.plan.n_scalers
        K = (w_post.shape[2] - fi) // S
        w_h = w_post[:, :, :fi]
        w_a = w_post[:, :, fi:].reshape(T, fo, S, K).permute(0, 2, 1, 3)
        id_slot = _identity_slot(self.plan.applied_scalers)
        if id_slot is not None:
            hcols = torch.zeros(T, S, fo, fi, dtype=dt, device=dev)
            hcols[:, id_slot] = w_h
            ops["w"] = torch.cat([w_a, hcols], dim=3).reshape(T, S * fo, K + fi)
        else:
            ops["w_a"] = w_a.reshape(T, S * fo, K)
            ops["w_h"] = w_h.contiguous()
        return ops

    def _operands(self, dev):
        plist = self._param_list()
        key = (dev, id(plist), plist[0].shape, plist[2].shape)
        cache = self.__dict__.setdefault("_opmap", {})
        if key not in cache:
            with torch.no_grad():
                sizes = [p.numel() for p in plist]
                ids = torch.arange(1, sum(sizes) + 1, dtype=torch.float64, device=dev).split(sizes)
                id_ops = self._assemble([i.view(p.shape) for i, p in zip(ids, plist)])
                names = list(id_ops)
                flat_ids = torch.cat([id_ops[k].reshape(-1) for k in names])
                pos = torch.nonzero(flat_ids).flatten()
                sel = (flat_ids[pos] - 1).long()
                shapes = [tuple(id_ops[k].shape) for k in names]
                native = None
                n_flat = sum(sizes)
                if dev.type == "cuda" and sel.numel() == n_flat and all(p.dtype == torch.float32 and p.is_contiguous() for p in plist):
                    starts = torch.zeros(len(sizes) + 1, dtype=torch.long, device=dev)
                    starts[1:] = torch.cumsum(torch.tensor(sizes, device=dev), 0)
                    gid = (flat_ids - 1).long()
                    which = torch.bucketize(gid.clamp(min=0), starts[1:], right=True)
                    map_param = torch.where(gid >= 0, which, torch.full_like(which, -1)).int()
                    map_off = torch.where(gid >= 0, gid - starts[which], torch.zeros_like(gid)).int()
                    inv = torch.empty(n_flat, dtype=torch.long, device=dev)
                    inv[sel] = pos
                    native = dict(ptr_table=torch.zeros(len(plist), dtype=torch.int64, device=dev), ptr_host=None, map_param=map_param,
                                  map_off=map_off, inv=inv, total=flat_ids.numel(), sizes=sizes, shapes=[tuple(p.shape) for p in plist])
                cache[key] = (names, shapes, pos, sel, flat_ids.numel(), [math.prod(shp) for shp in shapes], native)
        names, shapes, pos, sel, total, sizes, native = cache[key]
        if native is not None and all(p.is_cuda and p.is_contiguous() for p in plist):
            native.setdefault("op_sizes", sizes)
            native.setdefault("op_shapes", shapes)
            return dict(zip(names, _ops.assemble_operands(native, plist)))
        else:
            flat = torch.cat([p.reshape(-1) for p in plist])
            fused = flat.new_zeros(total).index_put((pos,), flat.index_select(0, sel))
        return {k: part.view(shp) for k, part, shp in zip(names, fused.split(sizes), shapes)}

    def _fused_towers(self, g, h, e, snorm_n):
        graph = as_dgn_graph(g, h.device)
        T, fi, fo = len(self.towers), self.input_tower, self.output_tower
        ops = self._operands(h.device)
        x_in = h if self.divide_input else h.repeat(1, T)
        if self.divide_input and _ops.pair_linear_supported(h, T, fi):
            pq = _ops.pair_linear(h, ops["w_sd"], ops["bias_sd"], T, fi)
        else:
            pq = node_linear(h, ops["w_sd"], ops["bias_sd"])
        m_edge, edge_type = _edge_term(graph, e, ops["w_edge"]) if self.edge_features else (None, None)
        b_p = ops["b_p"]
        S = self.plan.n_scalers
        N = h.shape[0]
        row_scale = snorm_n if self.graph_norm else None
        if "w" in ops:
            sc = _scale_table(graph, self.plan.applied_scalers, self._avg_log) if S > 1 else None
            needs_grad = torch.is_grad_enabled() and (h.requires_grad or any(q.requires_grad for q in self.parameters()))
            if (_ops.FUSED_FORWARD and not needs_grad and m_edge is None and h.is_cuda and self.divide_input
                    and _ops.fused_sweep_posttrans_supported(graph, self._kplan_x, T, x_in.shape[1], S, fo)):
                w_edge = graph.edge_weights(self._kplan_x, g.ndata["eig"])
                y = _ops.fused_sweep_posttrans_forward(graph, self._kplan_x, T, self._avg_log, w_edge, pq, x_in.contiguous(), ops["w"], sc, b_p,
                                                       row_scale)
                return self._towers_tail(y, ops)
            aggx = directional_aggregate(graph, self._kplan_x, self._avg_log, x_pair=pq, m_edge=m_edge, x_in=x_in,
                                         eig=g.ndata["eig"], n_towers=T, tower_major=True, edge_type=edge_type)
            bns = [t.batchnorm_h for t in self.towers]
            fused_tail = self.batch_norm and self.training and bn_tail_supported(bns, aggx, True, T * fo)
            if fused_tail and linear_combine_supported(aggx, ops["w"], S):
                rm, rv, nbt = self._linked_bn_stats(aggx.device)
                y = linear_combine_bn_tail(aggx, ops["w"], sc, b_p, row_scale, ops["bn_gamma"], ops["bn_beta"], rm, rv, nbt,
                                           bns[0].momentum, bns[0].eps)
                return _dropout(y, self.dropout, self.training)
            z = node_linear(aggx, ops["w"])
            if fused_tail:
                rm, rv, nbt = self._linked_bn_stats(z.device)
                y = combine_bn_tail(z, sc, b_p, row_scale, ops["bn_gamma"], ops["bn_beta"], rm, rv, nbt, bns[0].momentum, bns[0].eps)
                return _dropout(y, self.dropout, self.training)
            y = scale_combine(z, sc, b_p, row_scale)
        else:
            agg = directional_aggregate(graph, self._kplan, self._avg_log, x_pair=pq, m_edge=m_edge,
                                        x_in=x_in, eig=g.ndata["eig"], n_towers=T, tower_major=True, edge_type=edge_type)
            z = node_linear(agg, ops["w_a"])
            sc = _scale_table(graph, self.plan.applied_scalers, self._avg_log)
            y = scale_combine(z, sc, b_p, None)
            y = y + torch.bmm(x_in.view(N, T, fi).transpose(0, 1), ops["w_h"].transpose(1, 2)).transpose(0, 1).reshape(N, T * fo)
            if row_scale is not None:
                y = y * row_scale
        return self._towers_tail(y, ops)

    def _towers_tail(self, y, ops):
        if self.batch_norm:
            bns = [t.batchnorm_h for t in self.towers]
            if bn_tail_supported(bns, y, self.training):
                rm, rv, nbt = self._linked_bn_stats(y.device)
                y = bn_tail_fused(y, ops["bn_gamma"], ops["bn_beta"], rm, rv, nbt, bns[0].momentum, bns[0].eps, self.training)
            else:
                y = bn_tail(y, bns, self.training)
        return _dropout(y, self.dropout, self.training)

    def _whole_layer(self, g, h, snorm_n):
        T, fi, fo = len(self.towers), self.input_tower, self.output_tower
        if not (_ops.WHOLE_LAYER and self.training and torch.is_grad_enabled() and self.batch_norm and T > 1 and self.divide_input
                and not self.edge_features and 0 <= self.dropout < 1 and h.is_cuda and h.dtype == torch.float32 and h.dim() == 2
                and _identity_slot(self.plan.applied_scalers) is not None and self._fusable()
                and towers_layer_supported(T, fi, fo, self.plan.n_scalers, self._kplan_x.n_agg)):
            return None
        act = self.mixing_network._fused_act()
        bns = [t.batchnorm_h for t in self.towers]
        if act is None or act[0] != "leaky_relu" or self.mixing_network.linear.bias is None or not bn_tail_supported(bns, h, True, T * fo):
            return None
        eig = g.ndata["eig"]
        graph = as_dgn_graph(g, h.device)
        ops = self._operands(h.device)
        S = self.plan.n_scalers
        sc = _scale_table(graph, self.plan.applied_scalers, self._avg_log) if S > 1 else None
        rm, rv, nbt = self._linked_bn_stats(h.device)
        w_edge = graph.edge_weights(self._kplan_x, eig)
        mix = self.mixing_network.linear
        drop = _block_dropout(self, h)
        y = towers_layer(graph, self._kplan_x, self._avg_log, w_edge, h, snorm_n if self.graph_norm else None, sc, rm, rv, nbt,
                         ops["w_sd"], ops["bias_sd"], ops["w"], ops["b_p"], ops["bn_gamma"], ops["bn_beta"], mix.weight, mix.bias,
                         T, fi, fo, self.residual, bns[0].momentum, bns[0].eps, act[1], dropout=drop,
                         id_slot=_identity_slot(self.plan.applied_scalers))
        if drop is not None:
            _dropout_key_used(drop[1])
        return y

    def _block_layer(self, g, h, snorm_n):
        T, fi, fo = len(self.towers), self.input_tower, self.output_tower
        if not (_block_route_ok(self, h) and T > 1 and T <= 8 and self.divide_input and not self.edge_features and 0 <= self.dropout < 1
                and self._fusable()):
            return None
        act = self.mixing_network._fused_act()
        mix = self.mixing_network.linear
        if act is None or act[0] != "leaky_relu" or mix.bias is None:
            return None
        plist = self._param_list()
        if any(p is None for p in plist):
            return None
        graph = as_dgn_graph(g, h.device)
        if not _ops.block_layer_supported(graph, self.plan, 2, T, fi, fo, eval_only=not self.training):
            return None
        bns = [t.batchnorm_h for t in self.towers]
        rm, rv, nbt = self._linked_bn_stats(h.device)
        drop = _block_dropout(self, h)
        y = _ops.block_layer(graph, self.plan, self._avg_log, g.ndata["eig"], h, snorm_n if self.graph_norm else None, rm, rv, nbt,
                             (*plist, mix.weight, mix.bias), 2, T, fi, fo, self.residual, bns[0].momentum, bns[0].eps, act[1], training=self.training,
                             dropout=drop)
        if drop is not None:
            _dropout_key_used(drop[1])
        return y

    def _forward(self, g, h, e, snorm_n):
        h_in = h
        y = self._block_layer(g, h, snorm_n)
        if y is None:
            y = self._whole_layer(g, h, snorm_n)
        if y is not None:
            return y
        if self._fusable():
            h_cat = self._fused_towers(g, h, e, snorm_n)
        elif self.divide_input:
            h_cat = torch.cat([tower(g, h[:, n * self.input_tower:(n + 1) * self.input_tower], e, snorm_n)
                               for n, tower in enumerate(self.towers)], dim=1)
        else:
            h_cat = torch.cat([tower(g, h, e, snorm_n) for tower in self.towers], dim=1)
        if len(self.towers) > 1:
            return self.mixing_network(h_cat, residual=h_in if self.residual else None)
        return h_in + h_cat if self.residual else h_cat


class DGNLayer(nn.Module):

    def __init__(self, in_dim, out_dim, dropout, graph_norm, batch_norm, aggregators, scalers, avg_d, type_net,
                 residual, towers=5, divide_input=True, edge_features=None, edge_dim=None, pretrans_layers=1,
                 posttrans_layers=1):
# ... 19 lines not shown
```

dgn_amd/graph.py:

```python
from __future__ import annotations

import ctypes as C
import os
from typing import Dict, Optional, Tuple

import functools

import torch

from . import _lib
from .spec import EPS, AggPlan, Channel

HUB_THRESHOLD = 2048
HUB_CHUNK = 1024
NATIVE_BUILD = True
DC_CLASSES, DC_UNIT = _lib.DGN_DC_CLASSES, _lib.DGN_DC_UNIT
GRAPH_BLOCK_MAX_ROWS = 512
BLOCK_MAX_GAP = 52
DEFERRED_STATS = True


def _ptr(t: Optional[torch.Tensor]) -> Optional[int]:
    return None if t is None else t.data_ptr()

# ... 431 lines not shown
            if "_blk" not in self.__dict__ and torch.cuda.is_current_stream_capturing():
                enabled = False
            if enabled and "_blk" not in self.__dict__:
                self._closed_cuts()
            if enabled:
                cut, gap = self._blk
                ok = 0 < gap <= BLOCK_MAX_GAP
        if ok:
            self._c.blk_cut, self._c.blk_gap = cut.data_ptr(), gap
        else:
            self._c.blk_cut, self._c.blk_gap = None, 0
        self._ensure_graph_blocks(enabled)
        return ok

    def _ensure_graph_blocks(self, enabled: bool = True) -> bool:
        ok = False
        if enabled and self.src.is_cuda and self.num_src == self.num_nodes and self.n_hub == 0 and getattr(self, "_pad", None) is None \
                and self.row_base == 0 and self.num_edges > 3 * self.num_nodes:
            t = self.block_table(target_rows=1)
            if t is not None and t["max_rows"] <= GRAPH_BLOCK_MAX_ROWS and getattr(self, "_csc_ready", False) and hasattr(self, "csc_order"):
                self._closed_cuts()
                self._c.gblk_desc, self._c.n_gblk, self._c.gblk_rows = t["desc"].data_ptr(), t["n_blocks"], t["max_rows"]
                self._c.csc_order, self._c.dst_csr = self.csc_order.data_ptr(), self.dst_csr.data_ptr()
                ok = True
        if not ok:
            self._c.gblk_desc, self._c.n_gblk, self._c.gblk_rows, self._c.csc_order, self._c.dst_csr = None, 0, 0, None, None
        return ok

    def number_of_nodes(self) -> int:
        return self.num_nodes

    def number_of_edges(self) -> int:
        return self.num_edges

    @property
    def c_graph(self) -> _lib.DgnGraph:
        return self._c

    def to_slot_order(self, per_edge: torch.Tensor) -> torch.Tensor:
        return per_edge if self.eid is None else per_edge.index_select(0, self.eid)

    def _normalised_eig(self, eig: torch.Tensor) -> torch.Tensor:
        ent = getattr(self, "_eig_norm", None)
        if ent is not None and ent[0] is eig and ent[1] == eig._version:
            return ent[2]
        e = eig
        if e.device != self.device:
            e = e.to(self.device)
        if e.dtype != torch.float32 or e.dim() != 2 or e.stride(-1) != 1:
            e = e.float().contiguous()
        self._eig_norm = (eig, eig._version, e)
        return e

    def edge_weights(self, plan: AggPlan, eig: Optional[torch.Tensor] = None) -> Optional[torch.Tensor]:
        if plan.n_channels == 0:
            return None
        eig = self._normalised_eig(self.ndata["eig"] if eig is None else eig)
        key = (id(eig), eig._version, tuple(eig.shape), plan.channels)
        ent = self._wcache.get(key)
        if ent is None or ent[0] is not eig:
            w = compute_edge_weights(self, plan.channels, eig=eig)
            if len(self._wcache) >= 8:
                self._wcache.clear()
            self._wcache[key] = ent = (eig, w)
        return ent[1]


@functools.lru_cache(maxsize=64)
def _channel_array(channels: Tuple[Channel, ...]):
    arr = (_lib.DgnChannel * len(channels))()
    for i, (kind, col, alpha) in enumerate(channels):
        arr[i].kind, arr[i].eig_col, arr[i].alpha, arr[i].eps = kind, col, alpha, EPS
    return arr


def compute_edge_weights(graph: DGNGraph, channels: Tuple[Channel, ...], eig: Optional[torch.Tensor] = None,
                         eig_s_edge: Optional[torch.Tensor] = None, eig_d_edge: Optional[torch.Tensor] = None) -> torch.Tensor:
    lib = _lib.load()
    ref = eig if eig is not None else eig_s_edge
    if ref is None or not ref.is_cuda:
        raise _lib.DgnError("dgn_amd runs on the GPU only: eig must be a CUDA tensor")
    E = graph.num_edges
    w = torch.empty((len(channels), max(E, 1)), dtype=torch.float32, device=ref.device)
    ld = ref.stride(0) if ref.dim() == 2 and ref.shape[0] > 0 else ref.shape[-1]
    stream = _lib.stream_ptr(ref.device)
    for c0 in range(0, len(channels), _lib.DGN_MAX_CH):
        chunk = channels[c0:c0 + _lib.DGN_MAX_CH]
        for ch in chunk:
            if ch[1] >= ref.shape[-1]:
                raise IndexError(f"aggregator needs eig column {ch[1]} but eig has {ref.shape[-1]} columns")
        nbytes = lib.dgn_edge_weights_workspace_bytes(C.byref(graph.c_graph), len(chunk))
        ws = torch.empty(nbytes, dtype=torch.uint8, device=ref.device) if nbytes else None
        rc = lib.dgn_edge_weights(C.byref(graph.c_graph), _ptr(eig), _ptr(eig_s_edge), _ptr(eig_d_edge), ld, len(chunk),
                                  _channel_array(chunk), w[c0:].data_ptr(), w.stride(0), _ptr(ws), nbytes, stream)
        _lib.check(rc, "dgn_edge_weights")
    return w


def as_dgn_graph(g, device: Optional[torch.device] = None) -> DGNGraph:
    if isinstance(g, DGNGraph):
        return g
    dev = torch.device(device) if device is not None else torch.device("cuda", torch.cuda.current_device())
    if dev.type == "cuda" and dev.index is None:
        dev = torch.device("cuda", torch.cuda.current_device())
    cached = getattr(g, "_dgn_graph", None)
    if cached is not None and cached.device == dev:
        cached.ndata["eig"] = g.ndata["eig"]
        return cached
    edges = g.all_edges(order="eid") if hasattr(g, "all_edges") else g.edges()
    src, dst = edges[0], edges[1]
    out = DGNGraph(src.to(dev), dst.to(dev), g.number_of_nodes(), eig=g.ndata["eig"])
    if getattr(g, "batch_num_nodes", None) is not None:
        out.batch_num_nodes = g.batch_num_nodes
    try:
        g._dgn_graph = out
    except Exception:
        pass
    return out
```

dgn_amd/ops.py:

```python
from __future__ import annotations

import ctypes as C
import os
from typing import Optional

import torch

from . import _lib
from .graph import DGNGraph, _ptr
from .spec import EPS, AggPlan


DETERMINISTIC_BACKWARD = "auto"


def _two_phase_scatter(F: int) -> bool:
    return (F % 2 == 0) if DETERMINISTIC_BACKWARD == "auto" else bool(DETERMINISTIC_BACKWARD)


BLOCK_BACKWARD = os.environ.get("DGN_BLOCK_BACKWARD", "1") != "0"

_N_VALID = None


# ... 869 lines not shown
def _carve(sizes, device, buf=None):
    offs, total = _carve_offsets(sizes)
    if buf is None:
        buf = torch.empty(max(total, 1), dtype=torch.float32, device=device)
    return buf, [buf[o:o + n] for o, n in zip(offs, sizes)]


def _carve_ptrs(sizes, device, buf=None):
    offs, total = _carve_offsets(sizes)
    if buf is None:
        buf = torch.empty(max(total, 1), dtype=torch.float32, device=device)
    base = buf.data_ptr()
    return buf, [base + 4 * o if n else None for o, n in zip(offs, sizes)]


def _layer_workspace(L, nbytes, dev):
    ws = torch.empty(max(nbytes, 1), dtype=torch.uint8, device=dev)
    L.ws, L.ws_bytes = ws.data_ptr(), nbytes
    return ws


def _towers_saved_sizes(cfg, plan, N, n_y1, n_z):
    T, fi, fo = cfg[:3]
    return [N * 2 * T * fi, T * N * plan.n_agg * fi, N * T * fo, n_y1, n_z, T * fo, T * fo]


def _towers_struct(graph, plan, avg_log, w_edge, cfg, h, snorm, scale, w_sd, bias_sd, w_post, b_post, gamma, beta, w_mix, b_mix, bufs, use_mask,
                   aux, drop_mask, n_valid):
    T, fi, fo, S, residual, momentum, eps, slope, drop = cfg[:9]
    pq, aggx, y0, y1, z, mean, invstd = bufs
    spec = _spec_structs(plan, T, avg_log, h.shape[0] * plan.n_agg * fi)[0]
    L = _lib.DgnTowersLayer()
    cg = graph.c_graph
    L.graph, L.spec = C.pointer(cg), C.pointer(spec)
    L.w, L.ld_w, L.log_deg = _ptr(w_edge), (w_edge.stride(0) if w_edge is not None else 0), graph.log_deg.data_ptr()
    L.n_towers, L.f_in, L.f_out, L.n_scalers, L.residual = T, fi, fo, S, int(residual)
    L.momentum, L.eps, L.slope = float(momentum), float(eps), float(slope)
    L.h, L.snorm, L.scale = h.data_ptr(), _ptr(snorm), _ptr(scale)
    L.w_sd, L.bias_sd, L.w_post, L.b_post = w_sd.data_ptr(), bias_sd.data_ptr(), w_post.data_ptr(), b_post.data_ptr()
    L.bn_gamma, L.bn_beta = gamma.data_ptr(), beta.data_ptr()
    L.w_mix, L.b_mix = w_mix.data_ptr(), b_mix.data_ptr()
    L.pq, L.aggx, L.y0, L.y1 = pq.data_ptr(), aggx.data_ptr(), y0.data_ptr(), (y1.data_ptr() if y1.numel() else None)
    L.z, L.zmask = (None, z.data_ptr()) if use_mask else (z.data_ptr(), None)
    L.save_mean, L.save_invstd = mean.data_ptr(), invstd.data_ptr()
    L.agg_aux = _ptr(aux)
    if drop is not None:
        L.drop_p, L.drop_mask = drop[0], drop_mask.data_ptr()
    L.n_valid = _ptr(n_valid)
    return L, (cg, spec)


class _TowersLayer(torch.autograd.Function):
    @staticmethod
    def forward(ctx, graph, plan, avg_log, w_edge, cfg, h, snorm, scale, running_mean, running_var, nbt,
                w_sd, bias_sd, w_post, b_post, gamma, beta, w_mix, b_mix):
        lib = _lib.load()
        global LAST_DROPOUT_MASK
        T, fi, fo, S, residual, momentum, eps, slope, drop = cfg[:9]
        if not h.is_cuda:
            raise _lib.DgnError("towers_layer: CUDA tensors only (dgn_amd has no CPU path)")
        N, Fo = h.shape[0], T * fo
        dev = h.device
        h, w_sd, bias_sd, w_post, b_post = h.contiguous(), w_sd.contiguous(), bias_sd.contiguous(), w_post.contiguous(), b_post.contiguous()
        gamma, beta, w_mix, b_mix = gamma.contiguous(), beta.contiguous(), w_mix.contiguous(), b_mix.contiguous()
        n_y1 = 0 if FUSE_BN_MIXING and drop is None else N * Fo
        use_mask = n_y1 == 0 and (h.data_ptr() & 15) == 0 and bool(lib.dgn_towers_layer_zmask_supported(T, fo))
        n_z = (lib.dgn_linear_act_mask_bytes(N, Fo) + 3) // 4 if use_mask else N * Fo
        saved_buf, bufs = _carve(_towers_saved_sizes(cfg, plan, N, n_y1, n_z), dev)
        ctx.n_y1, ctx.n_z, ctx.use_mask = n_y1, n_z, use_mask
        out = torch.empty((N, Fo), dtype=torch.float32, device=dev)
        drop_mask = torch.empty(lib.dgn_dropout_mask_bytes(N * Fo), dtype=torch.uint8, device=dev) if drop is not None else None
        ctx.n_valid = _N_VALID
        L, keep = _towers_struct(graph, plan, avg_log, w_edge, cfg, h, snorm, scale, w_sd, bias_sd, w_post, b_post, gamma, beta, w_mix, b_mix, bufs,
                                 use_mask, None, drop_mask, ctx.n_valid)
        L.running_mean, L.running_var, L.out = running_mean.data_ptr(), running_var.data_ptr(), out.data_ptr()
        if nbt is not None:
            L.num_batches_tracked, L.n_nbt = nbt.data_ptr(), nbt.numel()
        if drop is not None:
            L.drop_seed, L.drop_offset = drop[1].data_ptr(), int(drop[2])
            LAST_DROPOUT_MASK = drop_mask
        n_aux = int(lib.dgn_towers_layer_agg_aux_bytes(C.byref(L))) if AGG_AUX else 0
        aux = torch.empty(n_aux, dtype=torch.uint8, device=dev) if n_aux else None
        L.agg_aux = _ptr(aux)
        ws = _layer_workspace(L, lib.dgn_towers_layer_forward_workspace_bytes(C.byref(L)), dev)
        _lib.check(lib.dgn_towers_layer_forward(C.byref(L), _lib.stream_ptr(dev)), "dgn_towers_layer_forward")
        ctx.save_for_backward(w_edge, h, snorm, scale, w_sd, bias_sd, w_post, b_post, gamma, beta, w_mix, b_mix, saved_buf, aux, drop_mask)
        ctx.graph, ctx.plan, ctx.avg_log, ctx.cfg = graph, plan, avg_log, cfg
        return out

    @staticmethod
    def backward(ctx, g_out):
        lib = _lib.load()
        w_edge, h, snorm, scale, w_sd, bias_sd, w_post, b_post, gamma, beta, w_mix, b_mix, saved_buf, aux, drop_mask = ctx.saved_tensors
        graph, plan, cfg = ctx.graph, ctx.plan, ctx.cfg
        T, fi, fo, S = cfg[:4]
        id_slot = cfg[9] if len(cfg) > 9 else None
        N, Fm, Fo = h.shape[0], T * fi, T * fo
        K = plan.n_agg * fi
        dev = h.device
        _, bufs = _carve(_towers_saved_sizes(cfg, plan, N, ctx.n_y1, ctx.n_z), dev, saved_buf)
        g_out = g_out.contiguous()
        graph.ensure_csc()
        graph.ensure_blocks(bool(BLOCK_BACKWARD))
        L, keep = _towers_struct(graph, plan, ctx.avg_log, w_edge, cfg, h, snorm, scale, w_sd, bias_sd, w_post, b_post, gamma, beta, w_mix, b_mix, bufs,
                                 ctx.use_mask, aux, drop_mask, ctx.n_valid)
        L.id_slot1 = 0 if id_slot is None else int(id_slot) + 1
        ws = _layer_workspace(L, lib.dgn_towers_layer_backward_workspace_bytes(C.byref(L)), dev)
        g_h = torch.empty((N, Fm), dtype=torch.float32, device=dev)
        n_ops = [2 * Fm * Fm, 2 * Fm, Fo, Fo, Fo, T * S * fo * K]
        n_flat = _up64(sum(n_ops))
        gbuf = torch.empty(n_flat + _up64(Fo * Fo) + Fo, dtype=torch.float32, device=dev)
        g_w_sd, g_bias_sd, g_b_post, g_gamma, g_beta, g_w_post = gbuf[:sum(n_ops)].split(n_ops)
        g_w_mix, g_b_mix = gbuf[n_flat:n_flat + Fo * Fo], gbuf[n_flat + _up64(Fo * Fo):]
        G = _lib.DgnTowersGrads(g_out=g_out.data_ptr(), g_h=g_h.data_ptr(), g_w_sd=g_w_sd.data_ptr(), g_bias_sd=g_bias_sd.data_ptr(),
                                g_w_post=g_w_post.data_ptr(), g_b_post=g_b_post.data_ptr(), g_gamma=g_gamma.data_ptr(),
                                g_beta=g_beta.data_ptr(), g_w_mix=g_w_mix.data_ptr(), g_b_mix=g_b_mix.data_ptr())
        _lib.check(lib.dgn_towers_layer_backward(C.byref(L), C.byref(G), _lib.stream_ptr(dev)), "dgn_towers_layer_backward")
        return (None, None, None, None, None, g_h, None, None, None, None, None, g_w_sd.view(2 * Fm, Fm), g_bias_sd, g_w_post.view(T, S * fo, K),
                g_b_post, g_gamma, g_beta, g_w_mix.view(Fo, Fo), g_b_mix)


def towers_layer(graph: DGNGraph, plan: AggPlan, avg_log: float, w_edge, h, snorm, scale, running_mean, running_var, num_batches_tracked,
                 w_sd, bias_sd, w_post, b_post, gamma, beta, w_mix, b_mix, n_towers: int, f_in: int, f_out: int, residual: bool,
                 momentum: float, eps: float, slope: float, dropout=None, id_slot=None) -> torch.Tensor:
    S = 1 if scale is None else scale.shape[1]
    scale, _, snorm = _flat_operands(scale, None, snorm)
    drop = None if dropout is None else (float(dropout[0]), dropout[1], int(dropout[2]))
    cfg = (n_towers, f_in, f_out, S, bool(residual), float(momentum), float(eps), float(slope), drop, (0 if S == 1 else id_slot))
    nbt = _kernel_counter(num_batches_tracked, 256)
    return _TowersLayer.apply(graph, plan, float(avg_log), w_edge, cfg, h, snorm, scale, running_mean, running_var, nbt,
                              w_sd, bias_sd, w_post.contiguous(), b_post, gamma, beta, w_mix, b_mix)



_DENSE_OK = {}


def dense_layer_supported(type_net: int, f_in: int, f_out: int, n_scalers: int, n_agg: int) -> bool:
    key = (type_net, f_in, f_out, n_scalers, n_agg)
    if key not in _DENSE_OK:
        _DENSE_OK[key] = bool(_lib.load().dgn_dense_layer_supported(*key))
    return _DENSE_OK[key]


DC_POSTTRANS = os.environ.get("DGN_DC_POSTTRANS", "1") != "0"
DC_MIN_NODES = int(os.environ.get("DGN_DC_MIN_NODES", "16384"))


def _degree_classes(graph, scale, fo, K):
    if not DC_POSTTRANS or scale is None or not scale.is_cuda or graph.num_nodes < DC_MIN_NODES:
        return None
    lib = _lib.load()
    if not (lib.dgn_dc_supported(K, fo) and lib.dgn_dc_supported(fo, K) and lib.dgn_dc_wgrad_supported(K, fo)):
        return None
    dc = graph.degree_classes()
    if dc is None:
        return None
    cache = graph.__dict__.setdefault("_dc_scale", {})
    key = scale.data_ptr()
    if key not in cache:
        cache[key] = (scale, scale.index_select(0, dc["rep"]).contiguous())
    return dc, cache[key][1]


def _dc_struct(dc):
    if dc is None:
        return None
    g, cls_scale = dc
    return _lib.DgnDegreeClasses(n_units=g["n_units"], vperm=g["vperm"].data_ptr(), unit_class=g["unit_class"].data_ptr(),
                                 present=g["present"].data_ptr(), scale=cls_scale.data_ptr())


DC_SPLIT = os.environ.get("DGN_DC_SPLIT", "1") != "0"


def dc_posttrans_split_supported(graph: DGNGraph, agg: torch.Tensor, fo: int, S: int) -> bool:
    if not (DC_SPLIT and DC_POSTTRANS and S > 1 and agg.is_cuda and agg.dtype == torch.float32
            and graph.num_nodes >= DC_MIN_NODES and getattr(graph, "_pad", None) is None and graph.num_src == graph.num_nodes):
        return False
    lib = _lib.load()
    K = agg.shape[1]
    if not lib.dgn_dc_supported(K, fo):
        return False
# ... 433 lines not shown
    if not training:
        return _block_layer_eval(graph, plan, float(avg_log), eig, cfg, h, snorm, rm, rv, params)
    if DIRECT_PARAM_GRADS and h.requires_grad:
        return _BlockLayer.apply(graph, plan, float(avg_log), eig, cfg, h, snorm, rm, rv, nbt, tuple(params))
    return _BlockLayer.apply(graph, plan, float(avg_log), eig, cfg, h, snorm, rm, rv, nbt, None, *params)



FUSED_FORWARD = os.environ.get("DGN_FUSED_FORWARD", "1") != "0"
AGG_AUX = os.environ.get("DGN_AGG_AUX", "1") != "0"


def fused_sweep_posttrans_supported(graph: DGNGraph, plan: AggPlan, n_towers: int, F: int, n_scalers: int, f_out: int) -> bool:
    lib = _lib.load()
    if len(plan.launches) != 1:
        return False
    spec = _spec_structs(plan, n_towers, 1.0, 0)[0]
    return bool(lib.dgn_layer_fused_supported(C.byref(graph.c_graph), C.byref(spec), F, n_scalers, f_out))


def fused_sweep_posttrans_forward(graph: DGNGraph, plan: AggPlan, n_towers: int, avg_log: float, w_edge, x_pair, x_in, weight, scale, bias,
                                  row_scale) -> torch.Tensor:
    lib = _lib.load()
    N, F = x_in.shape
    T = n_towers
    S = 1 if scale is None else scale.shape[1]
    fo = weight.shape[1] // S
    weight = weight.contiguous()
    spec = _spec_structs(plan, T, avg_log, 0)[0]
    msg = _msg_struct(F, x_pair[:, :F], x_pair[:, F:], None, x_in)
    y = torch.empty((N, T * fo), dtype=torch.float32, device=x_in.device)
    if row_scale is not None:
        row_scale = row_scale.reshape(-1).contiguous()
    stream = _lib.stream_ptr(x_in.device)
    rc = lib.dgn_layer_fused_forward(C.byref(graph.c_graph), C.byref(spec), C.byref(msg), _ptr(w_edge), w_edge.stride(0) if w_edge is not None else 0,
                                     graph.log_deg.data_ptr(), weight.data_ptr(), weight.stride(1), weight.stride(0), S, fo,
                                     _ptr(scale.contiguous() if scale is not None else None), _ptr(bias), _ptr(row_scale), y.data_ptr(), y.stride(0), stream)
    _lib.check(rc, "dgn_layer_fused_forward")
    return y


class _AssembleOperands(torch.autograd.Function):

    @staticmethod
    def forward(ctx, maps, *params):
        lib = _lib.load()
        ptrs = [p.data_ptr() for p in params]
        if ptrs != maps["ptr_host"]:
            maps["ptr_table"].copy_(torch.tensor(ptrs, dtype=torch.int64), non_blocking=False)
            maps["ptr_host"] = ptrs
        dev = params[0].device
        out = torch.empty(maps["total"], dtype=torch.float32, device=dev)
        stream = _lib.stream_ptr(dev)
        _lib.check(lib.dgn_assemble_params(maps["total"], maps["ptr_table"].data_ptr(), maps["map_param"].data_ptr(), maps["map_off"].data_ptr(),
                                           out.data_ptr(), stream), "dgn_assemble_params")
        ctx.maps = maps
        return tuple(part.view(shp) for part, shp in zip(out.split(maps["op_sizes"]), maps["op_shapes"]))

    @staticmethod
    def backward(ctx, *gs):
        maps = ctx.maps
        sizes, total = maps["op_sizes"], maps["total"]
        flat = None
        if all(g is not None and g.is_contiguous() and g.dtype == torch.float32 for g in gs):
            st, at = gs[0].untyped_storage(), gs[0].data_ptr()
            for g, n in zip(gs, sizes):
                if g.data_ptr() != at or g.untyped_storage().data_ptr() != st.data_ptr():
                    st = None
                    break
                at += 4 * n
            if st is not None and (gs[0].storage_offset() + total) * 4 <= st.nbytes():
                flat = torch.empty(0, dtype=torch.float32, device=gs[0].device).set_(st, gs[0].storage_offset(), (total,))
        if flat is None:
            dev = next(g.device for g in gs if g is not None)
            flat = torch.cat([(g.reshape(-1) if g is not None else torch.zeros(n, dtype=torch.float32, device=dev)) for g, n in zip(gs, sizes)])
        g_flat = flat.index_select(0, maps["inv"])
        return (None,) + tuple(part.view(shp) for part, shp in zip(g_flat.split(maps["sizes"]), maps["shapes"]))


def assemble_operands(maps, params):
    return _AssembleOperands.apply(maps, *params)


def _workspace(n_bytes: int, dtype: torch.dtype, dev) -> torch.Tensor:
    return torch.empty(max(n_bytes // dtype.itemsize, 1), dtype=dtype, device=dev)


def _wants_grad(scores: torch.Tensor) -> bool:
    return torch.is_grad_enabled() and scores.requires_grad


def _loss_backward(entry: str, g: torch.Tensor, g_loss: torch.Tensor) -> torch.Tensor:
    g_loss = g_loss.to(torch.float32).contiguous()
    out = torch.empty_like(g)
    rc = getattr(_lib.load(), entry)(g.shape[0], g.shape[1], g.data_ptr(), g.stride(0), g_loss.data_ptr(), out.data_ptr(), out.stride(0),
                                     _lib.stream_ptr(g.device))
    _lib.check(rc, entry)
    return out


class _BalancedCrossEntropy(torch.autograd.Function):
    @staticmethod
    def forward(ctx, scores, labels, n_classes, want_confusion, want_grad):
        lib = _lib.load()
        if not scores.is_cuda:
            raise _lib.DgnError("balanced_cross_entropy: CUDA tensors only (dgn_amd has no CPU path)")
        if scores.dim() != 2 or scores.shape[1] != n_classes or scores.dtype != torch.float32:
            raise ValueError(f"balanced_cross_entropy: scores must be float32 [N, {n_classes}], got {scores.dtype} {tuple(scores.shape)}")
        if labels.dtype != torch.int64 or labels.shape != (scores.shape[0],):
            raise ValueError("balanced_cross_entropy: labels must be int64 [N]")
        if scores.stride(1) != 1:
            scores = scores.contiguous()
        labels = labels.contiguous()
        N, dev = scores.shape[0], scores.device
        out = torch.empty(1 + n_classes, dtype=torch.float32, device=dev)
        g = torch.empty(N, n_classes, dtype=torch.float32, device=dev) if want_grad else None
        cm = torch.empty(n_classes, n_classes, dtype=torch.int64, device=dev) if want_confusion else None
        ws_bytes = lib.dgn_node_ce_workspace_bytes(N, n_classes)
        ws = _workspace(ws_bytes, torch.float64, dev)
        rc = lib.dgn_node_ce_forward(N, n_classes, scores.data_ptr(), _ld(scores), labels.data_ptr(), out.data_ptr(), out.data_ptr() + 4,
                                     _ptr(g), n_classes, _ptr(cm), ws.data_ptr(), ws_bytes, _lib.stream_ptr(dev))
        _lib.check(rc, "dgn_node_ce_forward")
        ctx.save_for_backward(g)
        ctx.set_materialize_grads(False)
        loss = out[0]
        if want_confusion:
            ctx.mark_non_differentiable(cm)
            return loss, cm
        return loss
# ... 432 lines not shown
```

include/dgn_hip.h:

```cpp
#ifndef DGN_HIP_H
#define DGN_HIP_H

#include <stddef.h>
#include <stdint.h>

#ifdef __cplusplus
extern "C" {
#endif

#define DGN_ABI_VERSION 38

#define DGN_MAX_AGG 16
#define DGN_MAX_CH 4
#define DGN_MAX_SCALERS 4

enum {
    DGN_OK = 0,
    DGN_ERR_INVALID = -1,
    DGN_ERR_WORKSPACE = -2,
    DGN_ERR_HIP = -3
};

enum {
    DGN_AGG_MEAN = 0,
    DGN_AGG_SUM = 1,
    DGN_AGG_MAX = 2,
    DGN_AGG_MIN = 3,
    DGN_AGG_STD = 4,
    DGN_AGG_VAR = 5,
    DGN_AGG_DIR_AV = 6,
    DGN_AGG_DIR_WSUM = 7,
    DGN_AGG_DIR_DX = 8,
    DGN_AGG_DIR_DX_NO_ABS = 9,
    DGN_AGG_X_IN = 10
};

enum {
    DGN_W_ABSNORM = 0,
    DGN_W_BALANCED = 1,
    DGN_W_SOFTMAX = 2
};

enum {
    DGN_SCALE_IDENTITY = 0,
    DGN_SCALE_AMPLIFICATION = 1,
    DGN_SCALE_ATTENUATION = 2
};

typedef struct DgnGraph {
    int64_t n_nodes;
    int64_t n_edges;
    const int32_t* indptr;
    const int32_t* src;
    int64_t n_hub;
    const int32_t* hub_rows;
    const int32_t* hub_chunk_ptr;
    int64_t n_chunks;
    const int32_t* chunk_hub;
    int32_t hub_threshold;
    int32_t hub_chunk;
    const int32_t* csc_ptr;
    const int32_t* csc_pos;
    int32_t max_in_degree;
// ... 8 lines not shown

typedef struct DgnChannel {
    int32_t kind;
    int32_t eig_col;
    float alpha;
    float eps;
} DgnChannel;

typedef struct DgnAggSpec {
    int32_t n_agg;
    int32_t agg_op[DGN_MAX_AGG];
    int32_t agg_ch[DGN_MAX_AGG];
    int32_t n_ch;
    int32_t n_scalers;
    int32_t scaler[DGN_MAX_SCALERS];
    float avg_log;
    float eps;
    int32_t n_towers;
    int32_t agg_total;
    int32_t agg_offset;
    int64_t tower_stride;
} DgnAggSpec;

typedef struct DgnMsg {
    int64_t F;
    const float* x_src;  int64_t ld_src;
    const float* x_dst;  int64_t ld_dst;
    const float* m_edge; int64_t ld_edge;
    const float* x_in;   int64_t ld_in;
    const int32_t* edge_type; int32_t n_edge_types;
    int32_t f_valid;
} DgnMsg;
int dgn_agg_f_valid_supported(const DgnAggSpec* spec);
#define DGN_MAX_EDGE_TABLE 8192

typedef struct DgnMsgGrad {
    float* g_src;  int64_t ld_src;
    float* g_dst;  int64_t ld_dst;
    float* g_edge; int64_t ld_edge;
    float* g_in;   int64_t ld_in;
    int32_t accumulate;
} DgnMsgGrad;

int dgn_abi_version(void);
size_t dgn_sizeof(const char* struct_name);
int dgn_set_option(const char* name, int64_t value);
int64_t dgn_get_option(const char* name);
const char* dgn_last_error(void);

size_t dgn_edge_weights_workspace_bytes(const DgnGraph* g, int32_t n_ch);
int dgn_edge_weights(const DgnGraph* g, const float* eig, const float* eig_s_edge, const float* eig_d_edge,
                     int64_t ld_eig, int32_t n_ch, const DgnChannel* ch, float* w, int64_t ld_w,
                     void* ws, size_t ws_bytes, void* stream);

size_t dgn_agg_workspace_bytes(const DgnGraph* g, const DgnAggSpec* spec, int64_t F);
int dgn_agg_forward(const DgnGraph* g, const DgnAggSpec* spec, const DgnMsg* msg, const float* w, int64_t ld_w,
                    const float* log_deg, float* out, int64_t ld_out, void* ws, size_t ws_bytes, void* stream);

size_t dgn_agg_aux_bytes(const DgnGraph* g, const DgnAggSpec* spec, const DgnMsg* msg);
int dgn_agg_forward_aux(const DgnGraph* g, const DgnAggSpec* spec, const DgnMsg* msg, const float* w, int64_t ld_w,
                        const float* log_deg, float* out, int64_t ld_out, unsigned char* aux, void* ws, size_t ws_bytes, void* stream);
int dgn_agg_backward_aux(const DgnGraph* g, const DgnAggSpec* spec, const DgnMsg* msg, const float* w, int64_t ld_w,
                         const float* log_deg, const float* g_out, int64_t ld_gout, const unsigned char* aux, const DgnMsgGrad* grads,
                         void* ws, size_t ws_bytes, void* stream);

size_t dgn_agg_backward_workspace_bytes(const DgnGraph* g, const DgnAggSpec* spec, int64_t F, int32_t deterministic);
size_t dgn_agg_edge_table_workspace_bytes(int64_t F, int32_t n_edge_types);
int dgn_agg_backward(const DgnGraph* g, const DgnAggSpec* spec, const DgnMsg* msg, const float* w, int64_t ld_w,
                     const float* log_deg, const float* g_out, int64_t ld_gout, const DgnMsgGrad* grads,
                     void* ws, size_t ws_bytes, void* stream);

int dgn_scale_combine_forward(int64_t n_nodes, int32_t n_towers, int32_t n_scalers, int32_t f_out, const float* z,
                              const float* scale, const float* bias, const float* row_scale, float* y, int64_t ld_y,
                              void* stream);
size_t dgn_scale_combine_backward_workspace_bytes(int64_t n_nodes, int32_t n_towers, int32_t f_out);
typedef struct DgnBnGrad {
    const float* g_out;
    const float* y;
    int64_t ld;
    const float* gamma;
    const float* beta;
    const float* mean;
    const float* invstd;
    const float* sums;
    int32_t relu;
    const int64_t* n_valid;
} DgnBnGrad;
int dgn_scale_combine_backward(int64_t n_nodes, int32_t n_towers, int32_t n_scalers, int32_t f_out, const float* g_y,
                               int64_t ld_gy, const float* scale, const float* row_scale, float* g_z, float* g_bias,
                               void* ws, size_t ws_bytes, const DgnBnGrad* bn, void* stream);

size_t dgn_bn_tail_workspace_bytes(int64_t n_rows, int32_t F);
int dgn_bn_tail_forward(int64_t n_rows, int32_t F, const float* x, int64_t ld, const float* gamma, const float* beta,
                        float* running_mean, float* running_var, float momentum, float eps, int32_t training,
                        int32_t relu, const float* residual, float* y, float* save_mean, float* save_invstd, void* ws,
                        size_t ws_bytes, const int64_t* n_valid, void* stream);
int dgn_bn_tail_backward(int64_t n_rows, int32_t F, const float* g_y, const float* x, int64_t ld, const float* gamma,
                         const float* beta, const float* save_mean, const float* save_invstd, int32_t relu, float* g_x,
                         float* g_gamma, float* g_beta, float* sums, void* ws, size_t ws_bytes, const int64_t* n_valid, void* stream);

int dgn_bias_act_forward(int64_t n_rows, int32_t F, const float* x, int64_t ld, const float* bias, int32_t act, float slope,
                         const float* residual, float* y, void* stream);
int dgn_bias_act_backward(int64_t n_rows, int32_t F, const float* g_y, const float* x, int64_t ld, const float* bias,
                          int32_t act, float slope, float* g_x, float* g_bias, void* ws, size_t ws_bytes, void* stream);

size_t dgn_dropout_mask_bytes(int64_t n_elems);
// ... 67 lines not shown
int dgn_gemm_wgrad(int64_t n_rows, int32_t k, int32_t n, const float* g, int64_t ldg, const float* x, int64_t ldx, float* dw,
                   int64_t lddw, float* dbias, void* ws, size_t ws_bytes, void* stream);

int dgn_layer_fused_supported(const DgnGraph* g, const DgnAggSpec* spec, int64_t F, int32_t n_scalers, int32_t f_out);
int dgn_layer_fused_forward(const DgnGraph* g, const DgnAggSpec* spec, const DgnMsg* msg, const float* w, int64_t ld_w,
                            const float* log_deg, const float* weight, int64_t ldw, int64_t stride_w, int32_t n_scalers,
                            int32_t f_out, const float* scale, const float* bias, const float* row_scale, float* y, int64_t ld_y,
                            void* stream);
size_t dgn_graph_build_workspace_bytes(int64_t n_nodes, int64_t n_edges);
int dgn_graph_build(int64_t n_nodes, int64_t n_edges, const int64_t* src, const int64_t* dst, int32_t* indptr, int32_t* src_csr,
                    int32_t* dst_csr, int64_t* eid, float* log_deg, int64_t* in_degree, int32_t* stats, int32_t hub_threshold,
                    void* ws, size_t ws_bytes, void* stream);
int dgn_graph_build_cuts(int64_t n_nodes, int64_t n_edges, const int32_t* src_csr, const int32_t* dst_csr, int32_t* blk_cut,
                         int32_t* gap_out, void* ws, size_t ws_bytes, void* stream);
int dgn_graph_build_csc(int64_t n_nodes, int64_t n_edges, const int32_t* src_csr, int32_t* csc_ptr, int32_t* csc_pos,
                        int32_t* csc_order, void* ws, size_t ws_bytes, void* stream);


typedef struct DgnTowersLayer {
    const DgnGraph* graph;
    const DgnAggSpec* spec;
    const float* w;
    int64_t ld_w;
    const float* log_deg;
    int32_t n_towers, f_in, f_out, n_scalers;
    int32_t residual;
    float momentum, eps, slope;
    const float* h;
    const float* snorm;
    const float* scale;
    const float* w_sd;  const float* bias_sd;
    const float* w_post; const float* b_post;
    const float* bn_gamma; const float* bn_beta;
    float* running_mean; float* running_var;
    const float* w_mix; const float* b_mix;
    float* pq; float* aggx; float* y0; float* save_mean; float* save_invstd; float* y1; float* z;
    float* out;
    void* ws; size_t ws_bytes;
    const int64_t* n_valid;
    unsigned char* zmask;
    unsigned char* agg_aux;
    float drop_p;
    const int64_t* drop_seed;
    uint64_t drop_offset;
    unsigned char* drop_mask;
    int32_t id_slot1;
    int64_t* num_batches_tracked;
    int32_t n_nbt;
} DgnTowersLayer;
typedef struct DgnTowersGrads {
    const float* g_out;
    float* g_h;
    float* g_w_sd; float* g_bias_sd; float* g_w_post; float* g_b_post; float* g_gamma; float* g_beta; float* g_w_mix; float* g_b_mix;
} DgnTowersGrads;
int dgn_assemble_params(int64_t n_out, const int64_t* param_ptrs, const int32_t* map_param, const int32_t* map_off, float* out, void* stream);

#define DGN_DC_CLASSES 32
#define DGN_DC_UNIT 64
typedef struct DgnDegreeClasses {
    int64_t n_units;
    const int32_t* vperm;
    const int32_t* unit_class;
    const int32_t* present;
    const float* scale;
} DgnDegreeClasses;
typedef struct DgnDcLayout {
    int32_t n_agg, f_pad, f_in, h_off, id_slot;
    int64_t ld;
} DgnDcLayout;
int dgn_dc_supported(int32_t k, int32_t n);
int dgn_dc_wgrad_supported(int32_t k, int32_t n);
int dgn_dc_fold(const DgnDegreeClasses* d, int32_t S, int32_t n, int32_t k, int32_t towers, const float* wf, const DgnDcLayout* layout ,
                float* wc, float* wct, void* stream);
int dgn_dc_gemm(const DgnDegreeClasses* d, int32_t k, int32_t n, int32_t towers, const float* a, int64_t lda, int64_t a_tower, const float* w,
                int64_t ldw, int64_t class_stride, int64_t w_tower, const float* bias, const float* row_scale, float* c, int64_t ldc,
                int64_t c_tower, int32_t stream_out, void* stream);
size_t dgn_dc_wgrad_workspace_bytes(int64_t n_units, int32_t k, int32_t n);
int dgn_dc_wgrad(const DgnDegreeClasses* d, int32_t S, int32_t k, int32_t n, const float* g, int64_t ldg, const float* x, int64_t ldx,
                 float* g_wf, int64_t ldw, const DgnDcLayout* layout , void* ws,
                 size_t ws_bytes, void* stream);

typedef struct DgnDenseLayer {
    const DgnGraph* graph;
    const DgnAggSpec* spec;
    const float* w;
    int64_t ld_w;
    const float* log_deg;
    int32_t type;
    int32_t f_in, f_out, n_scalers, n_agg;
    int32_t id_slot;
    int32_t residual;
    float momentum, eps;
    const float* h;
    const float* snorm;
    const float* scale;
    const float* w_pre;  const float* b_pre;
    const float* w_post; const float* b_post;
    const float* bn_gamma; const float* bn_beta;
    float* running_mean; float* running_var;
    float* hp; float* pq; float* agg; float* y; float* wf; float* wsd; float* save_mean; float* save_invstd;
    float* out;
    void* ws; size_t ws_bytes;
    const int64_t* n_valid;
    unsigned char* agg_aux;
    const DgnDegreeClasses* dc;
    int64_t* num_batches_tracked;
// ... 206 lines not shown
```

Before: 493.7 million edges/s.

## Fold parameter assembly and gradient scatter into existing kernel launches

Parameter assembly now runs inside the edge-weights flat kernel as extra blocks, which removes a separate small launch. In backward, the wgrad finalize kernels write each gradient directly into its flat parameter-gradient position. The deferred tower-stage finalize, the BD finalize and the bias copies are merged into a single tail launch, so the host-side index_select gather is skipped. This cuts several tiny kernel launches and one gather pass. In exchange it adds Python-side bookkeeping keyed by data pointers, plus a new ABI and a new options entry.

```diff
diff --git a/dgn_amd/csrc/dgn_abi.hip b/dgn_amd/csrc/dgn_abi.hip
--- a/dgn_amd/csrc/dgn_abi.hip
+++ b/dgn_amd/csrc/dgn_abi.hip
@@ -106,12 +106,13 @@
     {"ew_big_min", "DGN_EW_BIG_MIN", 1 << 19, false},
     {"ew_separate", "DGN_EW_SEPARATE", 0, true},
     {"ew_no_flat8", "DGN_EW_NO_FLAT8", 0, true},
+    {"fold_small", nullptr, 1, false},
 };
 std::atomic<int64_t> g_opt[OPT_COUNT];
 std::once_flag g_opt_once;
 void init_options() {
     for (int i = 0; i < OPT_COUNT; ++i) {
-        const char* e = getenv(kOpts[i].env);
+        const char* e = kOpts[i].env ? getenv(kOpts[i].env) : nullptr;
         g_opt[i].store(e ? (kOpts[i].presence ? 1 : atoll(e)) : kOpts[i].def, std::memory_order_relaxed);
     }
     if (getenv("DGN_NO_MIX_FUSED")) g_opt[OPT_NO_ZMASK].store(1, std::memory_order_relaxed);
diff --git a/dgn_amd/csrc/dgn_common.hpp b/dgn_amd/csrc/dgn_common.hpp
--- a/dgn_amd/csrc/dgn_common.hpp
+++ b/dgn_amd/csrc/dgn_common.hpp
@@ -17,7 +17,7 @@
 constexpr int kXcds = 8;
 
 void set_error(const char* fmt, ...);
-enum Opt { OPT_BLK_LDS_KB, OPT_BLK_MIN_NODES, OPT_BWD_ROWS_PER_WAVE, OPT_TILE_GEMM, OPT_TILE_WGRAD, OPT_NO_ZMASK, OPT_LINEAR_SMALL_MIN_WAVES, OPT_GRAPH_BWD_TILES, OPT_ODD_DIRECT, OPT_BN_FROM_WGRAD, OPT_MIX_BWD_FUSED, OPT_BLK_LDS_PAD_KB, OPT_LIN_WREG, OPT_BD_BWD_FUSED, OPT_BN_STATS_FUSED, OPT_EW_BIG_MIN, OPT_EW_SEPARATE, OPT_EW_NO_FLAT8, OPT_COUNT };
+enum Opt { OPT_BLK_LDS_KB, OPT_BLK_MIN_NODES, OPT_BWD_ROWS_PER_WAVE, OPT_TILE_GEMM, OPT_TILE_WGRAD, OPT_NO_ZMASK, OPT_LINEAR_SMALL_MIN_WAVES, OPT_GRAPH_BWD_TILES, OPT_ODD_DIRECT, OPT_BN_FROM_WGRAD, OPT_MIX_BWD_FUSED, OPT_BLK_LDS_PAD_KB, OPT_LIN_WREG, OPT_BD_BWD_FUSED, OPT_BN_STATS_FUSED, OPT_EW_BIG_MIN, OPT_EW_SEPARATE, OPT_EW_NO_FLAT8, OPT_FOLD_SMALL, OPT_COUNT };
 int64_t option(Opt o);
 int hip_fail(hipError_t e, const char* what);
 int zero_rows_async(float* p, int64_t rows, int64_t width, int64_t ld, hipStream_t stream);
@@ -70,12 +70,39 @@
 int combine_forward_stats(int64_t n_rows, int32_t k, int32_t n_towers, int32_t n_scalers, int32_t f_out, const float* a, int64_t stride_a,
                           const float* w, int64_t ldw, int64_t stride_w, const float* scale, const float* bias, const float* row_scale, float* y,
                           int64_t ld_y, double* part, size_t part_bytes, int* groups, void* stream);
+struct AssembleJob { int64_t n; const int64_t* ptrs; const int32_t* map_param; const int32_t* map_off; float* out; };
+__device__ __forceinline__ void assemble_element(const AssembleJob& j, int64_t i) {
+    if (i >= j.n) return;
+    const int q = j.map_param[i];
+    j.out[i] = q < 0 ? 0.f : reinterpret_cast<const float*>(j.ptrs[q])[j.map_off[i]];
+}
+struct ParamScatter { const int32_t* ppos; float* pflat; const float* obase; };
+__device__ __forceinline__ void store_operand(const ParamScatter& ps, float* q, float v) {
+    *q = v;
+    if (ps.ppos) {
+        const int j = ps.ppos[q - ps.obase];
+        if (j >= 0) ps.pflat[j] = v;
+    }
+}
+struct TsFinalize {
+    int T, n, k, slots, npad, kpad;
+    const float* part; float* dW; int64_t lddw, sdW; float* dbias; int64_t sdb;
+    float* pick; int pick_off, pick_w;
+    int blocks;
+    ParamScatter ps;
+};
+struct WgradTail {
+    TsFinalize ts;
+    ParamScatter ps;
+    const float* copy_src[2]; int copy_n[2];
+};
 int combine_backward_weight_bias_pick(int64_t n_rows, int32_t n_towers, int32_t n_scalers, int32_t f_out, int32_t k, const float* gy,
                                       int64_t stride_gy, const float* scale, const float* a, int64_t stride_a, float* dw, int64_t lddw,
-                                      int64_t stride_dw, float* g_sum, float* pick, int32_t pick_slot, void* ws, size_t ws_bytes, void* stream);
+                                      int64_t stride_dw, float* g_sum, float* pick, int32_t pick_slot, void* ws, size_t ws_bytes, void* stream,
+                                      TsFinalize* defer = nullptr);
 int bd_backward_both_launch(int64_t n_rows, int32_t n_towers, int32_t f_in, const float* g, const float* w, int64_t ldw, const float* x,
                             const float* add1, const float* add2, float* g_h, float* dw, int64_t lddw, float* dbias, void* ws, size_t ws_bytes,
-                            void* stream);
+                            void* stream, const WgradTail* tail = nullptr);
 }
 
 #define DGN_HIP_CHECK(expr)                                         \
diff --git a/dgn_amd/csrc/dgn_edge_weights.hip b/dgn_amd/csrc/dgn_edge_weights.hip
--- a/dgn_amd/csrc/dgn_edge_weights.hip
+++ b/dgn_amd/csrc/dgn_edge_weights.hip
@@ -180,6 +180,10 @@
 template <int FM>
 __device__ __forceinline__ void ew_flat_body(const EwParams& p, int64_t row64);
 __global__ __launch_bounds__(256) void ew_rows_flat(const EwParams p) { ew_flat_body<kFlatMax>(p, (int64_t)blockIdx.x * blockDim.x + threadIdx.x); }
+__global__ __launch_bounds__(256) void ew_rows_flat_assemble(const EwParams p, const lin::AssembleJob job, int ew_blocks) {
+    if ((int)blockIdx.x < ew_blocks) ew_flat_body<kFlatMax>(p, (int64_t)blockIdx.x * blockDim.x + threadIdx.x);
+    else lin::assemble_element(job, ((int64_t)blockIdx.x - ew_blocks) * blockDim.x + threadIdx.x);
+}
 __global__ __launch_bounds__(256) void ew_rows_flat8(const EwParams p) { ew_flat_body<8>(p, (int64_t)blockIdx.x * blockDim.x + threadIdx.x); }
 template <int FM>
 __device__ __forceinline__ void ew_flat_body(const EwParams& p, int64_t row64) {
@@ -428,9 +432,9 @@
     return ws_bytes_for(g);
 }
 
-extern "C" int dgn_edge_weights(const DgnGraph* g, const float* eig, const float* eig_s_edge, const float* eig_d_edge,
-                                int64_t ld_eig, int32_t n_ch, const DgnChannel* ch, float* w, int64_t ld_w, void* ws,
-                                size_t ws_bytes, void* stream_) {
+static int edge_weights_impl(const DgnGraph* g, const float* eig, const float* eig_s_edge, const float* eig_d_edge,
+                             int64_t ld_eig, int32_t n_ch, const DgnChannel* ch, float* w, int64_t ld_w, void* ws,
+                             size_t ws_bytes, void* stream_, const lin::AssembleJob* job, bool* job_done) {
     if (!g || !ch || !w) { set_error("null graph/channels/output"); return DGN_ERR_INVALID; }
     if (n_ch < 1 || n_ch > DGN_MAX_CH) { set_error("n_ch=%d outside 1..%d", n_ch, DGN_MAX_CH); return DGN_ERR_INVALID; }
     if (!eig && !(eig_s_edge && eig_d_edge)) { set_error("need eig, or eig_s_edge and eig_d_edge"); return DGN_ERR_INVALID; }
@@ -477,7 +481,13 @@
         const bool rows = g->max_in_degree == 0 || g->max_in_degree > kGroup;
         hipLaunchKernelGGL(ew_rows_small, dim3((unsigned)(nf + ng + (rows ? p.n_nodes : 0))), dim3(kWave), 0, stream, p, nf, ng);
     } else {
-    hipLaunchKernelGGL(ew_rows_flat, dim3((unsigned)((p.n_nodes + 255) / 256)), dim3(256), 0, stream, p);
+    const unsigned flat_blocks = (unsigned)((p.n_nodes + 255) / 256);
+    if (job && job->n > 0 && option(OPT_FOLD_SMALL) != 0) {
+        hipLaunchKernelGGL(ew_rows_flat_assemble, dim3(flat_blocks + (unsigned)((job->n + 255) / 256)), dim3(256), 0, stream, p, *job, (int)flat_blocks);
+        *job_done = true;
+    } else {
+        hipLaunchKernelGGL(ew_rows_flat, dim3(flat_blocks), dim3(256), 0, stream, p);
+    }
     if (g->max_in_degree == 0 || g->max_in_degree > kFlatMax)
     {
         if (big) hipLaunchKernelGGL(ew_rows_g16<kWave>, dim3((unsigned)((p.n_nodes + kWave - 1) / kWave)), dim3(kWave), 0, stream, p);
@@ -497,3 +507,21 @@
     DGN_HIP_CHECK(hipGetLastError());
     return DGN_OK;
 }
+
+extern "C" int dgn_edge_weights(const DgnGraph* g, const float* eig, const float* eig_s_edge, const float* eig_d_edge,
+                                int64_t ld_eig, int32_t n_ch, const DgnChannel* ch, float* w, int64_t ld_w, void* ws,
+                                size_t ws_bytes, void* stream) {
+    return edge_weights_impl(g, eig, eig_s_edge, eig_d_edge, ld_eig, n_ch, ch, w, ld_w, ws, ws_bytes, stream, nullptr, nullptr);
+}
+
+extern "C" int dgn_edge_weights_assemble(const DgnGraph* g, const float* eig, const float* eig_s_edge, const float* eig_d_edge,
+                                         int64_t ld_eig, int32_t n_ch, const DgnChannel* ch, float* w, int64_t ld_w, void* ws,
+                                         size_t ws_bytes, int64_t n_out, const int64_t* param_ptrs, const int32_t* map_param,
+                                         const int32_t* map_off, float* out, void* stream) {
+    if (n_out < 0 || n_out > INT32_MAX || (n_out > 0 && (!param_ptrs || !map_param || !map_off || !out))) { set_error("dgn_edge_weights_assemble: null or oversized assemble job"); return DGN_ERR_INVALID; }
+    const lin::AssembleJob job{n_out, param_ptrs, map_param, map_off, out};
+    bool done = false;
+    const int rc = edge_weights_impl(g, eig, eig_s_edge, eig_d_edge, ld_eig, n_ch, ch, w, ld_w, ws, ws_bytes, stream, &job, &done);
+    if (rc != DGN_OK) return rc;
+    return done ? DGN_OK : dgn_assemble_params(n_out, param_ptrs, map_param, map_off, out, stream);
+}
diff --git a/dgn_amd/csrc/dgn_linear.hip b/dgn_amd/csrc/dgn_linear.hip
--- a/dgn_amd/csrc/dgn_linear.hip
+++ b/dgn_amd/csrc/dgn_linear.hip
@@ -245,7 +245,7 @@
 }
 
 static int launch_wgrad(const char* fn, WgParams& p, float* dw, int64_t lddw, int64_t stride_dw, float* dbias, int64_t stride_dbias,
-                        void* ws, size_t ws_bytes, void* stream, float* pick = nullptr, int pick_off = 0, int pick_w = 0) {
+                        void* ws, size_t ws_bytes, void* stream, float* pick = nullptr, int pick_off = 0, int pick_w = 0, TsFinalize* defer = nullptr) {
     hipStream_t st = static_cast<hipStream_t>(stream);
     const int n = p.n, k = p.k, batch = p.T;
     const size_t need = dgn_linear_wgrad_workspace_bytes(p.M, k, n, batch);
@@ -259,8 +259,10 @@
     const hipError_t e = p.ex.gy ? launch_wgrad_expand(NT, KT, p, lds, st) : (p.g_mask ? launch_wgrad_gmask(NT, KT, p, lds, st) : launch_wgrad_plain(NT, KT, p, lds, st));
     DGN_HIP_CHECK(e);
     const int64_t total = (int64_t)batch * n * (dbias ? k + 1 : k);
-    hipLaunchKernelGGL(ts_wgrad_finalize, dim3((unsigned)((total + 63) / 64)), dim3(64 * wg::kSumWaves), 0, st, batch, n, k, p.groups,
-                       NT * 16, KT * 16, p.part, dw, lddw, stride_dw, dbias, stride_dbias, dbias ? pick : nullptr, pick_off, pick_w);
+    const TsFinalize fin{batch, n, k, p.groups, NT * 16, KT * 16, p.part, dw, lddw, stride_dw, dbias, stride_dbias, dbias ? pick : nullptr, pick_off, pick_w,
+                         (int)((total + 63) / 64), ParamScatter{}};
+    if (defer) { *defer = fin; return 0; }
+    hipLaunchKernelGGL(ts_wgrad_finalize, dim3((unsigned)fin.blocks), dim3(64 * wg::kSumWaves), 0, st, fin);
     DGN_HIP_CHECK(hipGetLastError());
     return 0;
 }
@@ -377,8 +379,9 @@
 int dgn::lin::combine_backward_weight_bias_pick(int64_t n_rows, int32_t n_towers, int32_t n_scalers, int32_t f_out, int32_t k, const float* gy,
                                                 int64_t stride_gy, const float* scale, const float* a, int64_t stride_a, float* dw, int64_t lddw,
                                                 int64_t stride_dw, float* g_sum, float* pick, int32_t pick_slot, void* ws, size_t ws_bytes,
-                                                void* stream) {
+                                                void* stream, TsFinalize* defer) {
     const char* fn = "dgn_linear_combine_backward_weight";
+    if (defer) defer->blocks = 0;
     if (g_sum && k % 16 == 0) { set_error("%s: the column sums ride in A's padding column (k %% 16 != 0)", fn); return -1; }
     const int n = n_scalers * f_out;
     if (!expand_ok(fn, n_rows, n_towers, n_scalers, f_out, gy, stride_gy, scale)) return -1;
@@ -394,5 +397,5 @@
     if (n_scalers == 1) { p.G = gy; p.sG = stride_gy; }
     else p.ex = ExpandSrc{gy, stride_gy, scale, n_scalers, f_out};
     if (pick && (!g_sum || pick_slot < 0 || pick_slot >= n_scalers)) { set_error("%s: pick needs g_sum and a scaler slot", fn); return -1; }
-    return launch_wgrad(fn, p, dw, lddw, stride_dw, g_sum, n, ws, ws_bytes, stream, pick, pick_slot * f_out, f_out);
-}
+    return launch_wgrad(fn, p, dw, lddw, stride_dw, g_sum, n, ws, ws_bytes, stream, pick, pick_slot * f_out, f_out, defer);
+}
diff --git a/dgn_amd/csrc/dgn_linear_bd.hip b/dgn_amd/csrc/dgn_linear_bd.hip
--- a/dgn_amd/csrc/dgn_linear_bd.hip
+++ b/dgn_amd/csrc/dgn_linear_bd.hip
@@ -418,11 +418,11 @@
     wg::wave_fold<NTW * 256>(lds, p.part, blockIdx.x, accw, [&](int q, int r) { return q * 256 + (4 * g + r) * 16 + m; });
 }
 
-static __global__ __launch_bounds__(64 * wg::kSumWaves) void bd_wgrad_finalize(int T, int fi, int FB, int slots, const float* __restrict__ part,
-                                                                               float* __restrict__ dW, int64_t lddw, float* __restrict__ dbias) {
-    __shared__ float red[wg::kSumWaves][64];
+struct BdFinalize { int T, fi, FB, slots; const float* part; float* dW; int64_t lddw; float* dbias; ParamScatter ps; };
+__device__ __forceinline__ void bd_wgrad_finalize_block(const BdFinalize& f, int64_t block, float (&red)[wg::kSumWaves][64]) {
+    const int T = f.T, fi = f.fi, FB = f.FB;
     const int Fm = T * fi, kk = Fm + 1, ntl = 2 * T * FB * FB;
-    const int64_t e = (int64_t)blockIdx.x * 64 + (threadIdx.x & 63);
+    const int64_t e = block * 64 + (threadIdx.x & 63);
     const bool live = e < (int64_t)2 * Fm * kk;
     int r = 0, c = 0, off = 0;
     bool diag = false;
@@ -434,10 +434,28 @@
         diag = c == Fm || (c >= t * fi && c < (t + 1) * fi);
         if (diag) off = (((t * 2 + j) * FB + (a >> 4)) * FB + (b >> 4)) * 256 + (a & 15) * 16 + (b & 15);
     }
-    const float v = wg::slot_sum16(part + off, (int64_t)ntl * 256, slots, diag, red);
+    const float v = wg::slot_sum16(f.part + off, (int64_t)ntl * 256, f.slots, diag, red);
     if (live && threadIdx.x < 64) {
-        if (c < Fm) dW[(int64_t)r * lddw + c] = v;
-        else if (dbias) dbias[r] = v;
+        if (c < Fm) store_operand(f.ps, f.dW + (int64_t)r * f.lddw + c, v);
+        else if (f.dbias) store_operand(f.ps, f.dbias + r, v);
+    }
+}
+static __global__ __launch_bounds__(64 * wg::kSumWaves) void bd_wgrad_finalize(BdFinalize a) {
+    __shared__ float red[wg::kSumWaves][64];
+    bd_wgrad_finalize_block(a, blockIdx.x, red);
+}
+static __global__ __launch_bounds__(64 * wg::kSumWaves) void wgrad_tail_finalize(WgradTail tl, BdFinalize bd, int n_bd) {
+    __shared__ float red[wg::kSumWaves][64];
+    const int b = blockIdx.x;
+    if (b < tl.ts.blocks) ts_wgrad_finalize_block(tl.ts, b, red);
+    else if (b < tl.ts.blocks + n_bd) bd_wgrad_finalize_block(bd, (int64_t)b - tl.ts.blocks, red);
+    else {
+#pragma unroll
+        for (int r = 0; r < 2; ++r)
+            for (int i = threadIdx.x; i < tl.copy_n[r]; i += blockDim.x) {
+                const int j = tl.ps.ppos[tl.copy_src[r] + i - tl.ps.obase];
+                if (j >= 0) tl.ps.pflat[j] = tl.copy_src[r][i];
+            }
     }
 }
 
@@ -498,11 +516,15 @@
     return 0;
 }
 
-int bd_finalize(const BdParams& p, float* dw, int64_t lddw, float* dbias, hipStream_t st) {
+int bd_finalize(const BdParams& p, float* dw, int64_t lddw, float* dbias, hipStream_t st, const WgradTail* tail = nullptr) {
     const int Fm = p.T * p.fi;
     const int64_t total = (int64_t)2 * Fm * (Fm + 1);
-    hipLaunchKernelGGL(bd_wgrad_finalize, dim3((unsigned)((total + 63) / 64)), dim3(64 * wg::kSumWaves), 0, st, p.T, p.fi, bd_blocks(p.T, p.fi), p.groups, p.part, dw,
-                       lddw, dbias);
+    const unsigned blocks = (unsigned)((total + 63) / 64);
+    const BdFinalize fin{p.T, p.fi, bd_blocks(p.T, p.fi), p.groups, p.part, dw, lddw, dbias, tail ? tail->ps : ParamScatter{}};
+    if (tail) {
+        const bool copy = tail->ps.ppos && tail->copy_n[0] + tail->copy_n[1] > 0;
+        hipLaunchKernelGGL(wgrad_tail_finalize, dim3(blocks + (unsigned)tail->ts.blocks + (copy ? 1u : 0u)), dim3(64 * wg::kSumWaves), 0, st, *tail, fin, (int)blocks);
+    } else hipLaunchKernelGGL(bd_wgrad_finalize, dim3(blocks), dim3(64 * wg::kSumWaves), 0, st, fin);
     DGN_HIP_CHECK(hipGetLastError());
     return DGN_OK;
 }
@@ -573,7 +595,7 @@
 namespace lin {
 int bd_backward_both_launch(int64_t n_rows, int32_t n_towers, int32_t f_in, const float* g, const float* w, int64_t ldw, const float* x,
                             const float* add1, const float* add2, float* g_h, float* dw, int64_t lddw, float* dbias, void* ws, size_t ws_bytes,
-                            void* stream) {
+                            void* stream, const WgradTail* tail) {
     const char* fn = "bd_backward_both";
     const int FB = bd_blocks(n_towers, f_in);
     const int Fm = n_towers * f_in;
@@ -596,7 +618,7 @@
     p.groups = (int)std::max<int64_t>(1, std::min<int64_t>(std::min<int64_t>(n_cus(), bd_wgrad_groups(n_rows)), (n_strips + waves - 1) / waves));
     hipStream_t st = static_cast<hipStream_t>(stream);
     DGN_HIP_CHECK(bd_launch(kBdBoth, p, waves * 64, lds, st));
-    return bd_finalize(p, dw, lddw, dbias, st);
-}
-}
-}
+    return bd_finalize(p, dw, lddw, dbias, st, tail);
+}
+}
+}
diff --git a/dgn_amd/csrc/dgn_linear_kernels.hpp b/dgn_amd/csrc/dgn_linear_kernels.hpp
--- a/dgn_amd/csrc/dgn_linear_kernels.hpp
+++ b/dgn_amd/csrc/dgn_linear_kernels.hpp
@@ -688,14 +688,11 @@
                                      [&](int q, int r) { return (16 * (q / KT) + 4 * mq + r) * (KT * 16) + 16 * (q % KT) + i16; });
 }
 
-static __global__ __launch_bounds__(64 * wg::kSumWaves) void ts_wgrad_finalize(int T, int n, int k, int slots, int npad, int kpad,
-                                                         const float* __restrict__ part, float* __restrict__ dW,
-                                                         int64_t lddw, int64_t sdW, float* __restrict__ dbias, int64_t sdb,
-                                                         float* __restrict__ pick = nullptr, int pick_off = 0, int pick_w = 0) {
-    __shared__ float red[wg::kSumWaves][64];
-    const int kk = dbias ? k + 1 : k;
-    const int64_t e = (int64_t)blockIdx.x * 64 + (threadIdx.x & 63);
-    const bool live = e < (int64_t)T * n * kk;
+__device__ __forceinline__ void ts_wgrad_finalize_block(const TsFinalize& a, int64_t block, float (&red)[wg::kSumWaves][64]) {
+    const int n = a.n, k = a.k;
+    const int kk = a.dbias ? k + 1 : k;
+    const int64_t e = block * 64 + (threadIdx.x & 63);
+    const bool live = e < (int64_t)a.T * n * kk;
     int t = 0, r = 0, c = 0;
     if (live) {
         t = (int)(e / ((int64_t)n * kk));
@@ -703,14 +700,18 @@
         r = rem / kk;
         c = rem - r * kk;
     }
-    const float v = wg::slot_sum16(part + (int64_t)t * slots * npad * kpad + (int64_t)r * kpad + c, (int64_t)npad * kpad, slots, live, red);
+    const float v = wg::slot_sum16(a.part + (int64_t)t * a.slots * a.npad * a.kpad + (int64_t)r * a.kpad + c, (int64_t)a.npad * a.kpad, a.slots, live, red);
     if (live && threadIdx.x < 64) {
-        if (c < k) dW[(int64_t)t * sdW + (int64_t)r * lddw + c] = v;
+        if (c < k) store_operand(a.ps, a.dW + (int64_t)t * a.sdW + (int64_t)r * a.lddw + c, v);
         else {
-            dbias[(int64_t)t * sdb + r] = v;
-            if (pick && r >= pick_off && r < pick_off + pick_w) pick[t * pick_w + r - pick_off] = v;
-        }
-    }
+            a.dbias[(int64_t)t * a.sdb + r] = v;
+            if (a.pick && r >= a.pick_off && r < a.pick_off + a.pick_w) store_operand(a.ps, a.pick + t * a.pick_w + r - a.pick_off, v);
+        }
+    }
+}
+static __global__ __launch_bounds__(64 * wg::kSumWaves) void ts_wgrad_finalize(TsFinalize a) {
+    __shared__ float red[wg::kSumWaves][64];
+    ts_wgrad_finalize_block(a, blockIdx.x, red);
 }
 
 constexpr bool linear_shape_ok(int NT, int KB, int mode) {
diff --git a/dgn_amd/csrc/dgn_towers.hip b/dgn_amd/csrc/dgn_towers.hip
--- a/dgn_amd/csrc/dgn_towers.hip
+++ b/dgn_amd/csrc/dgn_towers.hip
@@ -33,10 +33,7 @@
 
 __global__ __launch_bounds__(256) void assemble_params(int64_t n, const int64_t* __restrict__ ptrs, const int32_t* __restrict__ map_param,
                                                        const int32_t* __restrict__ map_off, float* __restrict__ out) {
-    const int64_t i = (int64_t)blockIdx.x * blockDim.x + threadIdx.x;
-    if (i >= n) return;
-    const int q = map_param[i];
-    out[i] = q < 0 ? 0.f : reinterpret_cast<const float*>(ptrs[q])[map_off[i]];
+    lin::assemble_element(lin::AssembleJob{n, ptrs, map_param, map_off, out}, (int64_t)blockIdx.x * blockDim.x + threadIdx.x);
 }
 
 __global__ __launch_bounds__(64) void mix_bn_finalize(int Fo, const float* __restrict__ dwx, const float* __restrict__ db, const float* __restrict__ w,
@@ -235,12 +232,44 @@
     return bwd_scratch(L, d).total;
 }
 
+namespace {
+__global__ __launch_bounds__(256) void scatter_params(int64_t n, const float* __restrict__ g_operands, const int32_t* __restrict__ pos, float* __restrict__ g_params) {
+    const int64_t i = (int64_t)blockIdx.x * blockDim.x + threadIdx.x;
+    if (i >= n) return;
+    const int j = pos[i];
+    if (j >= 0) g_params[j] = g_operands[i];
+}
+int towers_backward(const DgnTowersLayer* L, const DgnTowersGrads* G, const Dims& d, bool* params_done, void* stream);
+}
+
 extern "C" int dgn_towers_layer_backward(const DgnTowersLayer* L, const DgnTowersGrads* G, void* stream) {
     const char* fn = "dgn_towers_layer_backward";
     Dims d;
     if (!dims_of(L, d, fn)) return DGN_ERR_INVALID;
     if (!G) { set_error("%s: null grads", fn); return DGN_ERR_INVALID; }
+    if (G->param_pos) {
+        const float* lo = G->g_operands;
+        auto in = [&](const float* q, int64_t n) { return q && lo && q >= lo && q + n <= lo + G->n_operands; };
+        if (!G->g_params || G->n_operands <= 0 || G->n_operands > INT32_MAX || !in(G->g_w_sd, (int64_t)2 * d.Fm * d.Fm) || !in(G->g_bias_sd, 2 * d.Fm) ||
+            !in(G->g_w_post, (int64_t)d.T * d.S * d.fo * d.K) || !in(G->g_b_post, d.Fo) || !in(G->g_gamma, d.Fo) || !in(G->g_beta, d.Fo)) {
+            set_error("%s: param_pos needs g_params and every operand gradient inside [g_operands, g_operands + n_operands)", fn);
+            return DGN_ERR_INVALID;
+        }
+    }
     if (d.N == 0) return DGN_OK;
+    bool params_done = false;
+    DGN_TRY(towers_backward(L, G, d, &params_done, stream));
+    if (G->param_pos && !params_done) {
+        hipLaunchKernelGGL(scatter_params, dim3((unsigned)((G->n_operands + 255) / 256)), dim3(256), 0, static_cast<hipStream_t>(stream), G->n_operands,
+                           G->g_operands, G->param_pos, G->g_params);
+        DGN_HIP_CHECK(hipGetLastError());
+    }
+    return DGN_OK;
+}
+
+namespace {
+int towers_backward(const DgnTowersLayer* L, const DgnTowersGrads* G, const Dims& d, bool* params_done, void* stream) {
+    const char* fn = "dgn_towers_layer_backward";
     if (!G->g_out || !G->g_h || !G->g_w_sd || !G->g_bias_sd || !G->g_w_post || !G->g_b_post || !G->g_gamma || !G->g_beta || !G->g_w_mix ||
         !G->g_b_mix) { set_error("%s: null gradient buffer", fn); return DGN_ERR_INVALID; }
     if (!drop_ok(L, fn, false)) return DGN_ERR_INVALID;
@@ -255,6 +284,11 @@
     const bool bn_derived = fused_act && L->drop_p == 0.0f && !L->n_valid && option(OPT_BN_FROM_WGRAD) != 0;
     const bool mix_fused = bn_derived && L->zmask && (reinterpret_cast<uintptr_t>(L->zmask) & 15) == 0 && L->id_slot1 >= 1 && L->id_slot1 <= d.S && d.K % 16 != 0 && d.T <= 15 &&
                            (reinterpret_cast<uintptr_t>(L->y0) & 15) == 0 && dgn_linear_bnb_supported(d.Fo, d.Fo) && option(OPT_MIX_BWD_FUSED) != 0;
+    const float* res = L->residual ? G->g_out : nullptr;
+    const bool al = ((reinterpret_cast<uintptr_t>(G->g_h) | reinterpret_cast<uintptr_t>(G->g_out)) & 15) == 0;
+    const bool bd_path = use_bd(L, d) && al && ((reinterpret_cast<uintptr_t>(g_in) | reinterpret_cast<uintptr_t>(g_pq)) & 15) == 0;
+    const bool bd_both = bd_path && option(OPT_BD_BWD_FUSED) && d.fi <= 16 && (reinterpret_cast<uintptr_t>(L->h) & 15) == 0;
+    const bool fold = mix_fused && bd_both && option(OPT_FOLD_SMALL) != 0;
     if (mix_fused) {
         DGN_TRY(dgn_linear_wgrad_bn_act_mask(d.N, d.Fo, d.Fo, G->g_out, L->zmask, 2, L->slope, L->y0, f(s.dwx), d.Fo, G->g_b_mix, L->save_mean,
                                              L->save_invstd, nullptr, nullptr, ws + s.wg_mix, dgn_linear_wgrad_workspace_bytes(d.N, d.Fo, d.Fo, 1), stream));
@@ -300,9 +334,17 @@
     DGN_TRY(dgn_linear_combine_backward_input(d.N, d.T, d.S, d.fo, d.K, g_yr, d.N * d.fo, L->scale, L->w_post, d.K, (int64_t)d.S * d.fo * d.K,
                                               g_aggx, d.N * d.K, stream));
     float* g_sum = mix_fused ? f(s.g_sum) : nullptr;
+    lin::WgradTail tail{};
+    lin::TsFinalize& post_fin = tail.ts;
     DGN_TRY(lin::combine_backward_weight_bias_pick(d.N, d.T, d.S, d.fo, d.K, g_yr, d.N * d.fo, L->scale, L->aggx, d.N * d.K, G->g_w_post, d.K,
                                                    (int64_t)d.S * d.fo * d.K, g_sum, mix_fused ? G->g_b_post : nullptr, mix_fused ? L->id_slot1 - 1 : 0,
-                                                   ws + s.wg_post, dgn_linear_wgrad_workspace_bytes(d.N, d.K, d.S * d.fo, d.T), stream));
+                                                   ws + s.wg_post, dgn_linear_wgrad_workspace_bytes(d.N, d.K, d.S * d.fo, d.T), stream, fold ? &post_fin : nullptr));
+    if (fold && G->param_pos) {
+        tail.ps = lin::ParamScatter{G->param_pos, G->g_params, G->g_operands};
+        post_fin.ps = tail.ps;
+        tail.copy_src[0] = G->g_gamma; tail.copy_src[1] = G->g_beta;
+        tail.copy_n[0] = tail.copy_n[1] = d.Fo;
+    }
     const DgnMsg msg = sweep_msg(L, d);
     DgnMsgGrad gr{};
     gr.g_src = g_pq; gr.ld_src = 2 * d.Fm;
@@ -311,14 +353,13 @@
     gr.accumulate = 0;
     DGN_TRY(dgn_agg_backward_aux(L->graph, L->spec, &msg, L->w, L->ld_w, L->log_deg, g_aggx, d.K, L->agg_aux, &gr, ws + s.agg_ws,
                                  dgn_agg_backward_workspace_bytes(L->graph, L->spec, d.Fm, 1), stream));
-    const float* res = L->residual ? G->g_out : nullptr;
     static const bool no_add_epilogue = getenv("DGN_NO_ADD_EPILOGUE") != nullptr;
-    const bool al = ((reinterpret_cast<uintptr_t>(G->g_h) | reinterpret_cast<uintptr_t>(G->g_out)) & 15) == 0;
     const bool fused_add = !no_add_epilogue && al && (reinterpret_cast<uintptr_t>(g_in) & 15) == 0 && dgn_linear_add_supported(2 * d.Fm, d.Fm);
-    if (use_bd(L, d) && al && ((reinterpret_cast<uintptr_t>(g_in) | reinterpret_cast<uintptr_t>(g_pq)) & 15) == 0) {
-        if (option(OPT_BD_BWD_FUSED) && d.fi <= 16 && (reinterpret_cast<uintptr_t>(L->h) & 15) == 0) {
+    if (bd_path) {
+        if (bd_both) {
             DGN_TRY(lin::bd_backward_both_launch(d.N, d.T, d.fi, g_pq, L->w_sd, d.Fm, L->h, g_in, res, G->g_h, G->g_w_sd, d.Fm, G->g_bias_sd, ws + s.wg_sd,
-                                                 dgn_linear_bd_wgrad_workspace_bytes(d.N, d.T, d.fi), stream));
+                                                 dgn_linear_bd_wgrad_workspace_bytes(d.N, d.T, d.fi), stream, fold ? &tail : nullptr));
+            *params_done = fold && G->param_pos;
             return DGN_OK;
         }
         DGN_TRY(dgn_linear_bd_backward_input(d.N, d.T, d.fi, g_pq, L->w_sd, d.Fm, g_in, res, G->g_h, stream));
@@ -343,6 +384,8 @@
     return DGN_OK;
 }
 
+}
+
 extern "C" int dgn_assemble_params(int64_t n_out, const int64_t* param_ptrs, const int32_t* map_param, const int32_t* map_off, float* out,
                                    void* stream) {
     if (n_out < 0 || (n_out > 0 && (!param_ptrs || !map_param || !map_off || !out))) { set_error("dgn_assemble_params: null argument"); return DGN_ERR_INVALID; }
diff --git a/dgn_amd/dgn_layer.py b/dgn_amd/dgn_layer.py
--- a/dgn_amd/dgn_layer.py
+++ b/dgn_amd/dgn_layer.py
@@ -595,7 +595,7 @@
             ops["w_h"] = w_h.contiguous()
         return ops
 
-    def _operands(self, dev):
+    def _operands(self, dev, co_launch=None):
         plist = self._param_list()
         key = (dev, id(plist), plist[0].shape, plist[2].shape)
         cache = self.__dict__.setdefault("_opmap", {})
@@ -624,9 +624,13 @@
                                   map_off=map_off, inv=inv, total=flat_ids.numel(), sizes=sizes, shapes=[tuple(p.shape) for p in plist])
                 cache[key] = (names, shapes, pos, sel, flat_ids.numel(), [math.prod(shp) for shp in shapes], native)
         names, shapes, pos, sel, total, sizes, native = cache[key]
+        self.__dict__["_opmaps_used"] = None
         if native is not None and all(p.is_cuda and p.is_contiguous() for p in plist):
             native.setdefault("op_sizes", sizes)
             native.setdefault("op_shapes", shapes)
+            self.__dict__["_opmaps_used"] = native
+            if co_launch is not None:
+                native["co_launch"] = co_launch
             return dict(zip(names, _ops.assemble_operands(native, plist)))
         else:
             flat = torch.cat([p.reshape(-1) for p in plist])
@@ -705,7 +709,8 @@
             return None
         eig = g.ndata["eig"]
         graph = as_dgn_graph(g, h.device)
-        ops = self._operands(h.device)
+        fold = _ops._lib.options.fold_small != 0
+        ops = self._operands(h.device, co_launch=(lambda job: graph.edge_weights(self._kplan_x, eig, assemble=job)) if fold else None)
         S = self.plan.n_scalers
         sc = _scale_table(graph, self.plan.applied_scalers, self._avg_log) if S > 1 else None
         rm, rv, nbt = self._linked_bn_stats(h.device)
@@ -715,7 +720,7 @@
         y = towers_layer(graph, self._kplan_x, self._avg_log, w_edge, h, snorm_n if self.graph_norm else None, sc, rm, rv, nbt,
                          ops["w_sd"], ops["bias_sd"], ops["w"], ops["b_p"], ops["bn_gamma"], ops["bn_beta"], mix.weight, mix.bias,
                          T, fi, fo, self.residual, bns[0].momentum, bns[0].eps, act[1], dropout=drop,
-                         id_slot=_identity_slot(self.plan.applied_scalers))
+                         id_slot=_identity_slot(self.plan.applied_scalers), param_maps=self.__dict__.get("_opmaps_used"))
         if drop is not None:
             _dropout_key_used(drop[1])
         return y
diff --git a/dgn_amd/graph.py b/dgn_amd/graph.py
--- a/dgn_amd/graph.py
+++ b/dgn_amd/graph.py
@@ -507,14 +507,14 @@
         self._eig_norm = (eig, eig._version, e)
         return e
 
-    def edge_weights(self, plan: AggPlan, eig: Optional[torch.Tensor] = None) -> Optional[torch.Tensor]:
+    def edge_weights(self, plan: AggPlan, eig: Optional[torch.Tensor] = None, assemble: Optional[dict] = None) -> Optional[torch.Tensor]:
         if plan.n_channels == 0:
             return None
         eig = self._normalised_eig(self.ndata["eig"] if eig is None else eig)
         key = (id(eig), eig._version, tuple(eig.shape), plan.channels)
         ent = self._wcache.get(key)
         if ent is None or ent[0] is not eig:
-            w = compute_edge_weights(self, plan.channels, eig=eig)
+            w = compute_edge_weights(self, plan.channels, eig=eig, assemble=assemble)
             if len(self._wcache) >= 8:
                 self._wcache.clear()
             self._wcache[key] = ent = (eig, w)
@@ -530,7 +530,8 @@
 
 
 def compute_edge_weights(graph: DGNGraph, channels: Tuple[Channel, ...], eig: Optional[torch.Tensor] = None,
-                         eig_s_edge: Optional[torch.Tensor] = None, eig_d_edge: Optional[torch.Tensor] = None) -> torch.Tensor:
+                         eig_s_edge: Optional[torch.Tensor] = None, eig_d_edge: Optional[torch.Tensor] = None,
+                         assemble: Optional[dict] = None) -> torch.Tensor:
     lib = _lib.load()
     ref = eig if eig is not None else eig_s_edge
     if ref is None or not ref.is_cuda:
@@ -546,6 +547,13 @@
                 raise IndexError(f"aggregator needs eig column {ch[1]} but eig has {ref.shape[-1]} columns")
         nbytes = lib.dgn_edge_weights_workspace_bytes(C.byref(graph.c_graph), len(chunk))
         ws = torch.empty(nbytes, dtype=torch.uint8, device=ref.device) if nbytes else None
+        if assemble is not None and not assemble.get("done") and assemble["device"] == ref.device:
+            rc = lib.dgn_edge_weights_assemble(C.byref(graph.c_graph), _ptr(eig), _ptr(eig_s_edge), _ptr(eig_d_edge), ld, len(chunk),
+                                               _channel_array(chunk), w[c0:].data_ptr(), w.stride(0), _ptr(ws), nbytes, assemble["n_out"],
+                                               assemble["param_ptrs"], assemble["map_param"], assemble["map_off"], assemble["out"], stream)
+            _lib.check(rc, "dgn_edge_weights_assemble")
+            assemble["done"] = True
+            continue
         rc = lib.dgn_edge_weights(C.byref(graph.c_graph), _ptr(eig), _ptr(eig_s_edge), _ptr(eig_d_edge), ld, len(chunk),
                                   _channel_array(chunk), w[c0:].data_ptr(), w.stride(0), _ptr(ws), nbytes, stream)
         _lib.check(rc, "dgn_edge_weights")
diff --git a/dgn_amd/ops.py b/dgn_amd/ops.py
--- a/dgn_amd/ops.py
+++ b/dgn_amd/ops.py
@@ -945,10 +945,11 @@
 
 class _TowersLayer(torch.autograd.Function):
     @staticmethod
-    def forward(ctx, graph, plan, avg_log, w_edge, cfg, h, snorm, scale, running_mean, running_var, nbt,
+    def forward(ctx, graph, plan, avg_log, w_edge, cfg, pmaps, h, snorm, scale, running_mean, running_var, nbt,
                 w_sd, bias_sd, w_post, b_post, gamma, beta, w_mix, b_mix):
         lib = _lib.load()
         global LAST_DROPOUT_MASK
+        ctx.pmaps = pmaps
         T, fi, fo, S, residual, momentum, eps, slope, drop = cfg[:9]
         if not h.is_cuda:
             raise _lib.DgnError("towers_layer: CUDA tensors only (dgn_amd has no CPU path)")
@@ -1002,26 +1003,38 @@
         g_h = torch.empty((N, Fm), dtype=torch.float32, device=dev)
         n_ops = [2 * Fm * Fm, 2 * Fm, Fo, Fo, Fo, T * S * fo * K]
         n_flat = _up64(sum(n_ops))
-        gbuf = torch.empty(n_flat + _up64(Fo * Fo) + Fo, dtype=torch.float32, device=dev)
+        pmaps = ctx.pmaps if ctx.pmaps is not None and ctx.pmaps["total"] == sum(n_ops) else None
+        n_mix = _up64(Fo * Fo) + _up64(Fo)
+        n_par = sum(pmaps["sizes"]) if pmaps is not None else 0
+        gbuf = torch.empty(n_flat + n_mix + n_par, dtype=torch.float32, device=dev)
         g_w_sd, g_bias_sd, g_b_post, g_gamma, g_beta, g_w_post = gbuf[:sum(n_ops)].split(n_ops)
-        g_w_mix, g_b_mix = gbuf[n_flat:n_flat + Fo * Fo], gbuf[n_flat + _up64(Fo * Fo):]
+        g_w_mix, g_b_mix = gbuf[n_flat:n_flat + Fo * Fo], gbuf[n_flat + _up64(Fo * Fo):n_flat + _up64(Fo * Fo) + Fo]
         G = _lib.DgnTowersGrads(g_out=g_out.data_ptr(), g_h=g_h.data_ptr(), g_w_sd=g_w_sd.data_ptr(), g_bias_sd=g_bias_sd.data_ptr(),
                                 g_w_post=g_w_post.data_ptr(), g_b_post=g_b_post.data_ptr(), g_gamma=g_gamma.data_ptr(),
                                 g_beta=g_beta.data_ptr(), g_w_mix=g_w_mix.data_ptr(), g_b_mix=g_b_mix.data_ptr())
+        if pmaps is not None:
+            g_params = gbuf[n_flat + n_mix:]
+            G.param_pos, G.g_operands, G.n_operands, G.g_params = pmaps["param_pos"].data_ptr(), gbuf.data_ptr(), sum(n_ops), g_params.data_ptr()
         _lib.check(lib.dgn_towers_layer_backward(C.byref(L), C.byref(G), _lib.stream_ptr(dev)), "dgn_towers_layer_backward")
-        return (None, None, None, None, None, g_h, None, None, None, None, None, g_w_sd.view(2 * Fm, Fm), g_bias_sd, g_w_post.view(T, S * fo, K),
+        if pmaps is not None:
+            pmaps.setdefault("param_grads", {})[gbuf.data_ptr()] = g_params
+        return (None, None, None, None, None, None, g_h, None, None, None, None, None, g_w_sd.view(2 * Fm, Fm), g_bias_sd, g_w_post.view(T, S * fo, K),
                 g_b_post, g_gamma, g_beta, g_w_mix.view(Fo, Fo), g_b_mix)
 
 
 def towers_layer(graph: DGNGraph, plan: AggPlan, avg_log: float, w_edge, h, snorm, scale, running_mean, running_var, num_batches_tracked,
                  w_sd, bias_sd, w_post, b_post, gamma, beta, w_mix, b_mix, n_towers: int, f_in: int, f_out: int, residual: bool,
-                 momentum: float, eps: float, slope: float, dropout=None, id_slot=None) -> torch.Tensor:
+                 momentum: float, eps: float, slope: float, dropout=None, id_slot=None, param_maps=None) -> torch.Tensor:
     S = 1 if scale is None else scale.shape[1]
     scale, _, snorm = _flat_operands(scale, None, snorm)
     drop = None if dropout is None else (float(dropout[0]), dropout[1], int(dropout[2]))
     cfg = (n_towers, f_in, f_out, S, bool(residual), float(momentum), float(eps), float(slope), drop, (0 if S == 1 else id_slot))
     nbt = _kernel_counter(num_batches_tracked, 256)
-    return _TowersLayer.apply(graph, plan, float(avg_log), w_edge, cfg, h, snorm, scale, running_mean, running_var, nbt,
+    if param_maps is not None and "param_pos" not in param_maps:
+        ppos = torch.full((param_maps["total"],), -1, dtype=torch.int32, device=param_maps["inv"].device)
+        ppos[param_maps["inv"]] = torch.arange(param_maps["inv"].numel(), dtype=torch.int32, device=ppos.device)
+        param_maps["param_pos"] = ppos
+    return _TowersLayer.apply(graph, plan, float(avg_log), w_edge, cfg, param_maps, h, snorm, scale, running_mean, running_var, nbt,
                               w_sd, bias_sd, w_post.contiguous(), b_post, gamma, beta, w_mix, b_mix)
 
 
@@ -1561,8 +1574,13 @@
         dev = params[0].device
         out = torch.empty(maps["total"], dtype=torch.float32, device=dev)
         stream = _lib.stream_ptr(dev)
-        _lib.check(lib.dgn_assemble_params(maps["total"], maps["ptr_table"].data_ptr(), maps["map_param"].data_ptr(), maps["map_off"].data_ptr(),
-                                           out.data_ptr(), stream), "dgn_assemble_params")
+        co_launch = maps.pop("co_launch", None)
+        job = dict(n_out=maps["total"], param_ptrs=maps["ptr_table"].data_ptr(), map_param=maps["map_param"].data_ptr(),
+                   map_off=maps["map_off"].data_ptr(), out=out.data_ptr(), device=dev, done=False)
+        if co_launch is not None:
+            co_launch(job)
+        if not job["done"]:
+            _lib.check(lib.dgn_assemble_params(job["n_out"], job["param_ptrs"], job["map_param"], job["map_off"], job["out"], stream), "dgn_assemble_params")
         ctx.maps = maps
         return tuple(part.view(shp) for part, shp in zip(out.split(maps["op_sizes"]), maps["op_shapes"]))
 
@@ -1570,7 +1588,7 @@
     def backward(ctx, *gs):
         maps = ctx.maps
         sizes, total = maps["op_sizes"], maps["total"]
-        flat = None
+        flat, adjacent = None, False
         if all(g is not None and g.is_contiguous() and g.dtype == torch.float32 for g in gs):
             st, at = gs[0].untyped_storage(), gs[0].data_ptr()
             for g, n in zip(gs, sizes):
@@ -1580,10 +1598,16 @@
                 at += 4 * n
             if st is not None and (gs[0].storage_offset() + total) * 4 <= st.nbytes():
                 flat = torch.empty(0, dtype=torch.float32, device=gs[0].device).set_(st, gs[0].storage_offset(), (total,))
+                adjacent = True
         if flat is None:
             dev = next(g.device for g in gs if g is not None)
             flat = torch.cat([(g.reshape(-1) if g is not None else torch.zeros(n, dtype=torch.float32, device=dev)) for g, n in zip(gs, sizes)])
-        g_flat = flat.index_select(0, maps["inv"])
+        ready = maps.get("param_grads")
+        g_flat = ready.pop(flat.data_ptr(), None) if ready and adjacent else None
+        if ready:
+            ready.clear()
+        if g_flat is None:
+            g_flat = flat.index_select(0, maps["inv"])
         return (None,) + tuple(part.view(shp) for part, shp in zip(g_flat.split(maps["sizes"]), maps["shapes"]))
 
 
diff --git a/include/dgn_hip.h b/include/dgn_hip.h
--- a/include/dgn_hip.h
+++ b/include/dgn_hip.h
@@ -8,7 +8,7 @@
 extern "C" {
 #endif
 
-#define DGN_ABI_VERSION 38
+#define DGN_ABI_VERSION 39
 
 #define DGN_MAX_AGG 16
 #define DGN_MAX_CH 4
@@ -123,6 +123,10 @@
 int dgn_edge_weights(const DgnGraph* g, const float* eig, const float* eig_s_edge, const float* eig_d_edge,
                      int64_t ld_eig, int32_t n_ch, const DgnChannel* ch, float* w, int64_t ld_w,
                      void* ws, size_t ws_bytes, void* stream);
+int dgn_edge_weights_assemble(const DgnGraph* g, const float* eig, const float* eig_s_edge, const float* eig_d_edge,
+                              int64_t ld_eig, int32_t n_ch, const DgnChannel* ch, float* w, int64_t ld_w,
+                              void* ws, size_t ws_bytes, int64_t n_out, const int64_t* param_ptrs, const int32_t* map_param,
+                              const int32_t* map_off, float* out, void* stream);
 
 size_t dgn_agg_workspace_bytes(const DgnGraph* g, const DgnAggSpec* spec, int64_t F);
 int dgn_agg_forward(const DgnGraph* g, const DgnAggSpec* spec, const DgnMsg* msg, const float* w, int64_t ld_w,
@@ -296,6 +300,10 @@
     const float* g_out;
     float* g_h;
     float* g_w_sd; float* g_bias_sd; float* g_w_post; float* g_b_post; float* g_gamma; float* g_beta; float* g_w_mix; float* g_b_mix;
+    const int32_t* param_pos;
+    const float* g_operands;
+    int64_t n_operands;
+    float* g_params;
 } DgnTowersGrads;
 int dgn_assemble_params(int64_t n_out, const int64_t* param_ptrs, const int32_t* map_param, const int32_t* map_off, float* out, void* stream);
 
```

Result: no change. 495.9 million edges/s (median of 6 runs) (+0.4%).
